# by256/icsg3d

Hardware: AMD Instinct MI355X
Metric: voxel-grids/s (fwd+bwd) for 32^3 U-Net+VAE at batch 32: value = U-Net train step (BASELINE configs[1]); DFC-VAE step (configs[2]) in secondary; both per batch in unet_plus_vae (higher is better)
Workload: dtype f32

## Files before the change

icsg3d_amd/csrc/common.h:

```cpp
#pragma once
#include <hip/hip_runtime.h>
#include <hip/hip_ext.h>
#include <atomic>
#include <cstdint>
#include <cstdio>
#include <string>
#include <vector>

#include "up8.h"
#include "up125.h"

namespace ics {

extern std::atomic<long long> g_kernel_launches;
struct LaunchTimer {
  virtual void next(hipEvent_t* start, hipEvent_t* stop) = 0;
  virtual ~LaunchTimer() = default;
};
extern thread_local LaunchTimer* tl_launch_timer;
template <typename... P, typename... A>
inline void ics_launch(void (*kernel)(P...), dim3 grid, dim3 block, size_t shmem, hipStream_t st, A&&... args) {
  static_assert(sizeof...(P) == sizeof...(A), "kernel argument count");
  if (tl_launch_timer != nullptr) {
    hipEvent_t e0 = nullptr, e1 = nullptr;
    tl_launch_timer->next(&e0, &e1);
    hipExtLaunchKernelGGL(kernel, grid, block, (std::uint32_t)shmem, st, e0, e1, 0u, static_cast<P>(args)...);
  } else {
    hipLaunchKernelGGL(kernel, grid, block, shmem, st, static_cast<P>(args)...);
  }
}
#define ICS_LAUNCH(...)                                      \
  do {                                                       \
    ::ics::g_kernel_launches.fetch_add(1, std::memory_order_relaxed); \
    ::ics::ics_launch(__VA_ARGS__);                          \
  } while (0)

void set_error(const std::string& msg);
#define ICS_HIP(expr)                                                                     \
  do {                                                                                    \
    hipError_t _e = (expr);                                                               \
    if (_e != hipSuccess) {                                                               \
      ::ics::set_error(std::string(#expr) + " -> " + hipGetErrorString(_e) + " @" +       \
                       __FILE__ + ":" + std::to_string(__LINE__));                        \
      return -1;                                                                          \
    }                                                                                     \
  } while (0)
#define ICS_CHECK(cond, msg)                                                              \
  do {                                                                                    \
    if (!(cond)) {                                                                        \
      ::ics::set_error(std::string(msg) + " (" #cond ") @" + __FILE__ + ":" +             \
                       std::to_string(__LINE__));                                         \
      return -1;                                                                          \
    }                                                                                     \
  } while (0)
#define ICS_TRY(expr)                                                                     \
  do {                                                                                    \
    if ((expr) != 0) return -1;                                                           \
  } while (0)

enum Act : int { ACT_NONE = 0, ACT_RELU = 1, ACT_LRELU = 2 };
constexpr float kLeaky = 0.3f;
constexpr float kBnEps = 1e-3f;
constexpr float kKEps = 1e-7f;
constexpr float kPoolTieTol = 1e-5f;

__device__ __forceinline__ float act_fwd(float v, int act) {
  if (act == ACT_RELU) return fmaxf(v, 0.f);
  if (act == ACT_LRELU) return v > 0.f ? v : kLeaky * v;
  return v;
}
__device__ __forceinline__ float act_grad(float v, int act) {
  if (act == ACT_RELU) return v > 0.f ? 1.f : 0.f;
  if (act == ACT_LRELU) return v > 0.f ? 1.f : kLeaky;
  return 1.f;
}

struct ConvSrc {
  const float* p;
  const float* scale;
  const float* shift;
  int C;
  int up;
  int act;
  int bcast;
};

enum ConvFlags : int {
  CF_NO_REUSE = 1,
  CF_NO_WGRAD3 = 2,
  CF_NO_WGRAD3S = 4,
  CF_NO_FWD_SPLITK = 8,
  CF_NO_THIN_N = 16,
  CF_NO_UPSPLIT = 32,
  CF_NO_THIN_C = 64,
  CF_NO_COND_FOLD = 128,
  CF_NO_WINO = 256,
  CF_NO_WINO_WGRAD = 512,
  CF_NO_WINO64 = 1024,
  CF_NO_UP3 = 2048,
  CF_NO_THIN1_2STAGE = 4096,
  CF_NO_FAST_BNBWD = 8192,
  CF_NO_FUSED_HEAD = 16384,
  CF_NO_BWD_FOLD = 32768,
  CF_UP3_BIG_ALWAYS = 65536,
  CF_NO_WINOG = 262144,
  CF_NO_HEAD_BNFUSE = 524288,
  CF_NO_UP3N = 1 << 21,
  CF_NO_DGRAD_BNFUSE = 1 << 22,
  CF_NO_POOL_PRESUM = 1 << 23,
  CF_NO_HEAD_LABELS = 1 << 24,
  CF_NO_UP8 = 1 << 25,
  CF_UP8 = 1 << 26,
  CF_NO_UP125 = 1 << 27,
  CF_FORCE_UP125 = 1 << 28,
  CF_POOL125_V1 = 1 << 29,
  CF_ZBATCH = 1 << 20,
};
int conv_flags_from_env();

struct ConvGeom {
  int B, S, lgS;
  int Cin, Cout;
  int taps;
  int Kpad, Npad;
  int flags = 0;
};

struct BwdStat {
  const float* s = nullptr;
  const float* mean = nullptr;
  const float* rstd = nullptr;
  const float* scale = nullptr;
  const float* shift = nullptr;
  float* partial = nullptr;
  int post_act = ACT_NONE;
  int ld = 0;
  const float* abc = nullptr;
  float* db_partial = nullptr;
  const float* pool_d = nullptr;
  int pool_ld = 0;
  const unsigned char* pool_mask = nullptr;
};

int launch_conv_fwd(hipStream_t st, const ConvGeom& g, const ConvSrc* src, int nsrc,
                    const float* wpacked, const float* bias, float* out, int ldo, int pre_act,
                    float* stat_partial, int* stat_rows_per_block, int accumulate = 0,
                    float* splitk_ws = nullptr, size_t splitk_ws_floats = 0, const BwdStat* bwd = nullptr,
                    int* bwd_blocks = nullptr);
size_t conv_fwd_workspace_floats(const ConvGeom& g, const ConvSrc* src, int nsrc);
bool conv_fwd_up8_tile_ok(const ConvGeom& g);
bool conv_thin_c_ok(const ConvGeom& g, const ConvSrc& s0, int nsrc, int cin_log);
size_t conv_thin_c_wgrad_workspace_floats(const ConvGeom& g);
int launch_conv_wgrad_thin_c(hipStream_t st, const ConvGeom& g, const ConvSrc& s0, const float* dy, int ldy, float* dw,
                             int ldw, int row_pitch, float* ws, size_t ws_floats, int phase);
int launch_conv_fwd_thin_c(hipStream_t st, const ConvGeom& g, const ConvSrc& s0, int cin_log, int wstride,
                           const float* wp, const float* bias, float* out, int ldo, int pre_act, float* stat_partial,
                           int* rows_per_block, const float* pos_bias = nullptr);
int launch_conv_fwd_par(hipStream_t st, const ConvGeom& g_lowres, const ConvSrc& src, const float* wpar, float* out,
                        int ldo, const float* bias = nullptr, int pre_act = ACT_NONE, float* stat_partial = nullptr,
                        int* stat_blocks = nullptr);
int launch_pack_par(hipStream_t st, const float* w, int Cin_total, int Cout, int c_off, int Cu, float* dst, int Kpad,
                    int Npad);
int launch_pack_fwd_sub(hipStream_t st, const float* w, int taps, int Cin_total, int Cout, int c_off, int Csub,
                        float* dst, int Kpad, int Npad);
int launch_conv_wgrad(hipStream_t st, const ConvGeom& g, const ConvSrc* src, int nsrc,
                      const float* dy, int ldy, float* dw, int ldw, float* workspace,
                      size_t workspace_floats, int sub_rows = 0, int row_pitch = 0, int row_off = 0,
                      int phase = 0);
const char* conv_last_kernel_id();
void conv_set_last_kernel_id(const char* id);
int launch_pack_sub(hipStream_t st, const float* w, int taps, int Cin_total, int Cout, int c_off, int Csub,
                    int flip, float* dst, int Kpad, int Npad);
size_t conv_wgrad_workspace_floats(const ConvGeom& g, const ConvSrc* src, int nsrc);
int conv_fwd_rows_per_block(const ConvGeom& g);
int launch_conv_wgrad_ablate(hipStream_t st, const ConvGeom& g, const ConvSrc* src, const float* dy, int ldy,
                             float* workspace, int ablate);
int launch_conv_fwd_ablate(hipStream_t st, const ConvGeom& g, const ConvSrc* src, int nsrc, const float* wp,
                           float* out, int ldo, int ablate);
int launch_pack_fwd(hipStream_t st, const float* w, int K, int N, float* dst, int Kpad, int Npad,
                    int k_off, int n_off, int zero_first, int cin_log = 0, int cin_phys = 0);
void* pack_table_record_begin();
int pack_table_record_end(void* handle, std::vector<unsigned char>* bytes, int* njobs, unsigned* nblocks);
int launch_pack_table(hipStream_t st, const void* d_jobs, int njobs, unsigned nblocks);
int launch_materialize_input(hipStream_t st, const ConvSrc* src, int nsrc, int Cin, int CinG, int B, int S,
                             float* out);
int launch_pack_bwd(hipStream_t st, const float* w, int taps, int Cin, int Cout, float* dst,
                    int Kpad, int Npad, int cout_total, int co_off, int zero_first);

bool conv_wino_ok(const ConvGeom& g, const ConvSrc* src, int nsrc);
size_t conv_wino_weight_floats(int Cin, int Cout);
int launch_conv_fwd_wino(hipStream_t st, const ConvGeom& g, const ConvSrc& s0, const float* wt, const float* bias,
                         float* out, int ldo, int pre_act, float* stat_partial, int* rows_per_block, int accumulate,
                         int layout, const BwdStat* bwd = nullptr, int* bwd_blocks = nullptr);
int launch_pack_wino(hipStream_t st, const float* w, int Cin_total, int Cout, int c_off, int Csub, int bwd, float* dst,
                     int layout = 0);
int conv_wino_layout(const ConvGeom& g);
bool conv_wino64_ok(const ConvGeom& g, const ConvSrc* src, int nsrc);
int launch_conv_fwd_wino64(hipStream_t st, const ConvGeom& g, const ConvSrc& s0, const float* wt, const float* bias,
                           float* out, int ldo, int pre_act, float* stat_partial, int* rows_per_block, int accumulate,
                           const BwdStat* bwd = nullptr, int* bwd_blocks = nullptr);
bool conv_wino_wgrad_ok(const ConvGeom& g, const ConvSrc* src, int nsrc);
size_t conv_wino_wgrad_workspace_floats(const ConvGeom& g);
int launch_conv_wgrad_wino(hipStream_t st, const ConvGeom& g, const ConvSrc& s0, const float* dy, int ldy, float* dw,
                           int ldw, float* ws, size_t ws_floats, int sub_rows, int row_pitch, int row_off, int phase);
bool conv_up3_ok(const ConvGeom& g, const ConvSrc& s0);
size_t conv_up3_weight_floats(int Cu, int Cout);
int launch_pack_up3(hipStream_t st, const float* w, int Cin_total, int Cout, int c_off, int Cu, float* dst);
int launch_conv_fwd_up3(hipStream_t st, const ConvGeom& g, const ConvSrc& s0, const float* wt, const float* bias,
                        float* out, int ldo, int pre_act, float* stat_partial, int* stat_blocks, int accumulate);
bool conv_winog_ok(const ConvGeom& g, const ConvSrc* src, int nsrc);
bool conv_winog_wgrad_ok(const ConvGeom& g, const ConvSrc* src, int nsrc);
size_t conv_winog_weight_floats(int Cin, int Cout);
void conv_winog_scratch_floats(const ConvGeom& g, size_t* v, size_t* m, size_t* z);
int launch_conv_fwd_winog(hipStream_t st, const ConvGeom& g, const ConvSrc& s0, const float* wg, const float* bias, float* out,
                          int ldo, int pre_act, float* stat_partial, int* rows_per_block, float* v_scratch, float* m_scratch,
                          float* vt_keep);
int launch_conv_wgrad_winog(hipStream_t st, const ConvGeom& g, const float* vt, const float* dy, int ldy, float* dw, int ldw,
                            int row_pitch, int row_off, float* z_scratch, float* m_scratch);
int launch_gemm_zbatch(hipStream_t st, int nz, int M, int K, int N, const float* A, const float* Wp, float* out, int flags);
int wgrad_zbatch_splits(int nz, int M, int K, int N);
int launch_wgrad_zbatch(hipStream_t st, int nz, int M, int K, int N, const float* x, const float* dy, float* ws, int ksplit);
int launch_pack_up125(hipStream_t st, const float* w, int Cin_total, int N, int c_off, int Cu, float* dst);
int launch_pack_up125_pieces(hipStream_t st, const float* w, int Cin_total, int N, int c_off, int Cu, float* dst);
bool conv_up3n_ok(const ConvGeom& g, const ConvSrc& s0);
size_t conv_up3n_weight_floats(int Cu, int Cout);
int launch_pack_up3n(hipStream_t st, const float* w, int Cin_total, int Cout, int c_off, int Cu, float* dst);
int launch_conv_fwd_up3n(hipStream_t st, const ConvGeom& g, const ConvSrc& s0, const float* wt, const float* bias, float* out,
                         int ldo, int pre_act, float* stat_partial, int* stat_blocks);
int launch_wgrad_reduce_splits(hipStream_t st, const float* ws, int nsplit, size_t n_elems, int N, float* dw, int ldw,
                               int sub_rows, int row_pitch, int row_off);

}
```

icsg3d_amd/csrc/conv_igemm.hip:

```cpp
#include "common.h"

#ifndef ICS_GEMM_DEEP_FWD_MIN
#define ICS_GEMM_DEEP_FWD_MIN 1
#endif
#ifndef ICS_GEMM_DEEP_MIN
#define ICS_GEMM_DEEP_MIN 3
#endif
#ifndef ICS_GEMM_DEEP
#define ICS_GEMM_DEEP 1
#endif

#include <algorithm>
#include <type_traits>
#include <cstdlib>
#include <cstring>
#include <vector>

namespace ics {

typedef float f32x16 __attribute__((ext_vector_type(16)));
typedef float v4f __attribute__((ext_vector_type(4)));

#ifndef ICS_KLDA
#define ICS_KLDA 36
#endif
constexpr int kLDA = ICS_KLDA;

__device__ __forceinline__ int xcd_swizzle(int bid, int nblk) {
  const int xcd = bid & 7, q = nblk >> 3, r = nblk & 7;
  return (xcd < r ? xcd * (q + 1) : r * (q + 1) + (xcd - r) * q) + (bid >> 3);
}

static thread_local const char* g_last_kernel_id = "";
const char* conv_last_kernel_id() { return g_last_kernel_id; }
void conv_set_last_kernel_id(const char* id) { g_last_kernel_id = id; }
static const char* tf(bool b) { return b ? "true" : "false"; }

int conv_flags_from_env() {
  int f = 0;
  if (getenv("ICSG3D_NO_REUSE")) f |= CF_NO_REUSE;
  if (getenv("ICSG3D_NO_WGRAD3")) f |= CF_NO_WGRAD3;
  if (getenv("ICSG3D_NO_WGRAD3S")) f |= CF_NO_WGRAD3S;
  if (getenv("ICSG3D_NO_FWD_SPLITK")) f |= CF_NO_FWD_SPLITK;
  if (getenv("ICSG3D_NO_THIN_N")) f |= CF_NO_THIN_N;
  if (getenv("ICSG3D_NO_UPSPLIT")) f |= CF_NO_UPSPLIT;
  if (getenv("ICSG3D_NO_THIN_C")) f |= CF_NO_THIN_C;
  if (getenv("ICSG3D_NO_COND_FOLD")) f |= CF_NO_COND_FOLD;
  if (getenv("ICSG3D_NO_WINO")) f |= CF_NO_WINO;
  if (getenv("ICSG3D_NO_WINO_WGRAD")) f |= CF_NO_WINO_WGRAD;
  if (getenv("ICSG3D_NO_WINO64")) f |= CF_NO_WINO64;
  if (getenv("ICSG3D_NO_UP3")) f |= CF_NO_UP3;
  if (getenv("ICSG3D_NO_THIN1_2STAGE")) f |= CF_NO_THIN1_2STAGE;
  if (getenv("ICSG3D_NO_FAST_BNBWD")) f |= CF_NO_FAST_BNBWD;
  if (getenv("ICSG3D_NO_FUSED_HEAD")) f |= CF_NO_FUSED_HEAD;
  if (getenv("ICSG3D_NO_BWD_FOLD")) f |= CF_NO_BWD_FOLD;
  if (getenv("ICSG3D_NO_WINOG")) f |= CF_NO_WINOG;
  if (getenv("ICSG3D_NO_HEAD_BNFUSE")) f |= CF_NO_HEAD_BNFUSE;
  if (getenv("ICSG3D_NO_UP3N")) f |= CF_NO_UP3N;
  if (getenv("ICSG3D_NO_DGRAD_BNFUSE")) f |= CF_NO_DGRAD_BNFUSE;
  if (getenv("ICSG3D_NO_POOL_PRESUM")) f |= CF_NO_POOL_PRESUM;
  if (getenv("ICSG3D_NO_HEAD_LABELS")) f |= CF_NO_HEAD_LABELS;
  if (getenv("ICSG3D_NO_UP8")) f |= CF_NO_UP8;
  if (getenv("ICSG3D_NO_UP125")) f |= CF_NO_UP125;
  if (getenv("ICSG3D_FORCE_UP125")) f |= CF_FORCE_UP125;
  if (getenv("ICSG3D_POOL125_V1")) f |= CF_POOL125_V1;
  { const char* e = getenv("ICSG3D_UP3_BIG_MIN_WG"); if (e && *e && strtoul(e, nullptr, 10) <= 1) f |= CF_UP3_BIG_ALWAYS; }
  return f;
}
struct DevOnce {
  bool done[64] = {false};
  bool need(int* dev) {
    int d = 0;
    if (hipGetDevice(&d) != hipSuccess || d < 0 || d >= 64) { *dev = -1; return true; }
    *dev = d;
    return !done[d];
  }
  void mark(int dev) { if (dev >= 0) done[dev] = true; }
};

static int identity_affine(const float** ones, const float** zeros) {
  constexpr int kN = 16384;
  static float* buf[64] = {nullptr};
  int dev = 0;
  ICS_HIP(hipGetDevice(&dev));
  ICS_CHECK(dev >= 0 && dev < 64, "device index out of range");
  if (!buf[dev]) {
    float* p = nullptr;
    ICS_HIP(hipMalloc(&p, 2 * kN * sizeof(float)));
    std::vector<float> h(2 * kN, 0.f);
    for (int i = 0; i < kN; ++i) h[i] = 1.f;
    ICS_HIP(hipMemcpy(p, h.data(), 2 * kN * sizeof(float), hipMemcpyHostToDevice));
    buf[dev] = p;
  }
  *ones = buf[dev];
  *zeros = buf[dev] + kN;
  return 0;
}
static int fix_src(ConvSrc& s) {
  if (s.scale == nullptr) {
    ICS_CHECK(s.C <= 16384, "source wider than the identity-affine buffer");
    ICS_TRY(identity_affine(&s.scale, &s.shift));
    s.act = ACT_NONE;
  }
  return 0;
}

struct RowPos {
  int b, z, y, x;
};
__device__ __forceinline__ RowPos decode_row(int m, int S, int lg) {
  RowPos r;
  r.x = m & (S - 1);
  r.y = (m >> lg) & (S - 1);
  r.z = (m >> (2 * lg)) & (S - 1);
  r.b = m >> (3 * lg);
  return r;
}

__device__ __forceinline__ size_t src_voxel(const ConvSrc& s, int b, int z, int y, int x, int S) {
  if (s.up) {
    const int Sh = S >> 1;
    return ((((size_t)b * Sh + (z >> 1)) * Sh + (y >> 1)) * Sh + (x >> 1)) * (size_t)s.C;
  }
  return ((((size_t)b * S + z) * S + y) * S + x) * (size_t)s.C;
}

__host__ __device__ __forceinline__ float act_slope_of(int act) {
  return act == ACT_RELU ? 0.f : (act == ACT_LRELU ? kLeaky : 1.f);
}
__device__ __forceinline__ float act_apply(float v, float slope) {
  return fmaxf(v, v * slope);
}
template <bool NOACT>
__device__ __forceinline__ v4f affine_only_or_act4(v4f v, v4f sc, v4f sh, float slope);
__device__ __forceinline__ v4f affine_act4(v4f v, v4f sc, v4f sh, float slope) {
  v4f r;
  r.x = act_apply(fmaf(v.x, sc.x, sh.x), slope); r.y = act_apply(fmaf(v.y, sc.y, sh.y), slope);
  r.z = act_apply(fmaf(v.z, sc.z, sh.z), slope); r.w = act_apply(fmaf(v.w, sc.w, sh.w), slope);
  return r;
}
template <bool NOACT>
__device__ __forceinline__ v4f affine_only_or_act4(v4f v, v4f sc, v4f sh, float slope) {
  if (!NOACT) return affine_act4(v, sc, sh, slope);
  v4f r;
  r.x = fmaf(v.x, sc.x, sh.x); r.y = fmaf(v.y, sc.y, sh.y); r.z = fmaf(v.z, sc.z, sh.z); r.w = fmaf(v.w, sc.w, sh.w);
  return r;
}
__device__ __forceinline__ unsigned voxel_off(int b, int z, int y, int x, int S, int u, int C) {
  const int Ss = S >> u;
  return ((((unsigned)b * Ss + (z >> u)) * Ss + (y >> u)) * Ss + (x >> u)) * (unsigned)C;
}
__device__ __forceinline__ int clampi(int v, int hi) { return min(max(v, 0), hi); }

__device__ __forceinline__ ConvSrc pick_src(const ConvSrc& s0, const ConvSrc& s1, bool first) {
  ConvSrc s;
  s.p = first ? s0.p : s1.p;
  s.scale = first ? s0.scale : s1.scale;
  s.shift = first ? s0.shift : s1.shift;
  s.C = first ? s0.C : s1.C;
  s.up = first ? s0.up : s1.up;
  s.act = first ? s0.act : s1.act;
  s.bcast = first ? s0.bcast : s1.bcast;
  return s;
}

__device__ __forceinline__ float gather_scalar(const ConvSrc& s0, const ConvSrc& s1, int ci, int b,
                                               int z, int y, int x, int S) {
  const bool first = ci < s0.C;
  const ConvSrc s = pick_src(s0, s1, first);
  const int cl = first ? ci : ci - s0.C;
  float v;
  if (s.bcast > 0) {
    v = s.p[(size_t)b * s.bcast + (cl % s.bcast)];
  } else {
    v = s.p[src_voxel(s, b, z, y, x, S) + cl];
  }
  if (s.scale) v = act_fwd(fmaf(v, s.scale[cl], s.shift[cl]), s.act);
  return v;
}

template <int WM, int WN, int TM, int TN, bool VEC, int ABL = 0, bool AFF = true, bool UP = true, bool THIN = false,
          bool REUSE = false, bool PAR = false, bool NOACT = false, bool FOLD = false, bool UP8 = false>
__global__ __launch_bounds__(256, FOLD ? 2 : ((REUSE && PAR) ? 3 : 1)) void conv_fwd_kernel(ConvGeom g, ConvSrc s0, ConvSrc s1,
                                                        const float* __restrict__ wp,
                                                        const float* __restrict__ bias,
                                                        float* __restrict__ out, int ldo, int pre_act,
                                                        float* __restrict__ stat_partial, int gridM,
                                                        int gridN, int accumulate, BwdStat bs, Up8Geom u8) {
  constexpr int BM = WM * TM * 32, BN = WN * TN * 32;
  constexpr int B_FLOATS = 32 * BN;
  constexpr int RA = BM / 32;
  constexpr int RS = BM / 8;
  constexpr int NB = BN / 32;
  extern __shared__ __attribute__((aligned(16))) float smem[];
  const int A_FLOATS = (REUSE ? BM + (BM >> g.lgS) + 1 : BM) * kLDA;
  float* As = smem;
  constexpr int NABUF = 1;
  float* Bs = smem + NABUF * A_FLOATS;

  const int t = threadIdx.x, lane = t & 63, wave = t >> 6;
  const int wm = wave / WN, wn = wave % WN;
  const int li = lane & 31, lh = lane >> 5;
  const int sw = xcd_swizzle(blockIdx.x, gridM * gridN);
  const int mb = sw / gridN, nb = sw % gridN;
  const int S = g.S, lg = g.lgS;
  const int M = g.B << (3 * lg);
  const int n0 = nb * BN;
  const int nchunks = g.Kpad >> 5;
  const int cpt = (VEC && !THIN) ? (g.Cin >> 5) : 1;
  const int cls = PAR ? (int)blockIdx.y : 0;
  const int pz = cls >> 2, py = (cls >> 1) & 1, px = cls & 1;
  if (PAR) wp += (size_t)cls * g.Kpad * g.Npad;
  const bool zbatch = (g.flags & CF_ZBATCH) != 0;
  if (zbatch) {
    s0.p += (size_t)blockIdx.z * (size_t)M * (size_t)s0.C;
    wp += (size_t)blockIdx.z * (size_t)g.Kpad * (size_t)g.Npad;
    out += (size_t)blockIdx.z * (size_t)M * (size_t)ldo;
  }
  const int zsplit = zbatch ? 1 : (int)gridDim.z, zidx = zbatch ? 0 : (int)blockIdx.z;

  const int mrow_base = mb * BM + (VEC ? (t >> 3) : (t >> 5));
  const float slope0 = act_slope_of(s0.act), slope1 = act_slope_of(s1.act);
  const float pre_slope = act_slope_of(pre_act);

  unsigned rmask[RA];
  int rvh[RA];
  if (VEC) {
#pragma unroll
    for (int r = 0; r < RA; ++r) {
      const int m = mrow_base + 32 * r;
      const RowPos rp = decode_row(m, S, lg);
      unsigned mk = 0;
      if (m < M) {
        if (PAR) {
#pragma unroll
          for (int tp = 0; tp < 8; ++tp) {
            const int zz = rp.z + (tp >> 2) + pz - 1, yy = rp.y + ((tp >> 1) & 1) + py - 1, xx = rp.x + (tp & 1) + px - 1;
            const bool ok = (unsigned)zz < (unsigned)S && (unsigned)yy < (unsigned)S && (unsigned)xx < (unsigned)S;
            mk |= (ok ? 1u : 0u) << tp;
          }
#pragma unroll
          for (int gz = 0; gz < 4; ++gz) {
            const int zz = rp.z + (gz >> 1) + pz - 1, yy = rp.y + (gz & 1) + py - 1;
            mk |= (((unsigned)zz < (unsigned)S && (unsigned)yy < (unsigned)S) ? 1u : 0u) << (8 + gz);
          }
        } else if (g.taps == 27) {
          const unsigned zm = (rp.z > 0 ? 1u : 0u) | 2u | (rp.z < S - 1 ? 4u : 0u);
          const unsigned ym = (rp.y > 0 ? 1u : 0u) | 2u | (rp.y < S - 1 ? 4u : 0u);
          const unsigned xm = (rp.x > 0 ? 1u : 0u) | 2u | (rp.x < S - 1 ? 4u : 0u);
#pragma unroll
          for (int tp = 0; tp < 27; ++tp)
            mk |= (((zm >> (tp / 9)) & (ym >> ((tp / 3) % 3)) & (xm >> (tp % 3))) & 1u) << tp;
        } else {
          mk = 1u;
        }
      }
      mk |= ((unsigned)(rp.z & 1) << 29) | ((unsigned)(rp.y & 1) << 28) | ((unsigned)(rp.x & 1) << 27);
      rmask[r] = mk;
      const int Sh = S >> 1;
      rvh[r] = ((rp.b * Sh + (rp.z >> 1)) * Sh + (rp.y >> 1)) * Sh + (rp.x >> 1);
    }
  }

  v4f ra4[RA];
  float ras[RS];
  v4f rb[NB];

  unsigned bofs[NB];
#pragma unroll
  for (int r = 0; r < NB; ++r) {
    const int idx = t + 256 * r;
    bofs[r] = (unsigned)((idx / BN) * g.Npad + n0 + idx % BN) * 16u;
  }
  auto load_b = [&](int krow4) {
    const char* wrow = reinterpret_cast<const char*>(wp) + (size_t)krow4 * (size_t)g.Npad * 16;
#pragma unroll
    for (int r = 0; r < NB; ++r) rb[r] = *reinterpret_cast<const v4f*>(wrow + bofs[r]);
  };
  auto store_b = [&](int buf) {
    float* Bw = Bs + buf * B_FLOATS;
#pragma unroll
    for (int r = 0; r < NB; ++r) *reinterpret_cast<v4f*>(Bw + (t + 256 * r) * 4) = rb[r];
  };
  unsigned rowB0[RA], rowB1[RA];
  if (VEC) {
#pragma unroll
    for (int r = 0; r < RA; ++r) {
      rowB0[r] = (unsigned)(mrow_base + 32 * r) * (unsigned)s0.C * 4u;
      rowB1[r] = (unsigned)(mrow_base + 32 * r) * (unsigned)s1.C * 4u;
    }
  }
  auto load_a_group = [&](int gzy, int cc) {
    const int ci0 = cc << 5;
    const int dz = PAR ? (gzy >> 1) + pz - 1 : gzy / 3 - 1, dy = PAR ? (gzy & 1) + py - 1 : gzy % 3 - 1;
    const bool first = ci0 < s0.C;
    const char* sp = reinterpret_cast<const char*>(first ? s0.p : s1.p);
    const float* sscale = first ? s0.scale : s1.scale;
    const float* sshift = first ? s0.shift : s1.shift;
    const int sC = first ? s0.C : s1.C, su = first ? s0.up : s1.up;
    const float slope = first ? slope0 : slope1;
    const int cl = (first ? ci0 : ci0 - s0.C) + (t & 7) * 4;
    const v4f sc = *reinterpret_cast<const v4f*>(sscale + cl);
    const v4f sh = *reinterpret_cast<const v4f*>(sshift + cl);
    const int sdelta = (dz * S + dy) * S;
    const unsigned goffb = (unsigned)(sdelta * sC + cl) * 4u;
    const int Sh = S >> 1;
#pragma unroll
    for (int r = 0; r < RA; ++r) {
      const unsigned mk = rmask[r];
      const bool inb = (mk >> (PAR ? 8 + gzy : gzy * 3 + 1)) & 1u;
      unsigned offb = (first ? rowB0[r] : rowB1[r]) + goffb;
      if (UP) {
        const int ez = (dz + (int)((mk >> 29) & 1u)) >> 1;
        const int ey = (dy + (int)((mk >> 28) & 1u)) >> 1;
        const unsigned up_b = ((unsigned)(rvh[r] + (ez * Sh + ey) * Sh) * (unsigned)sC + (unsigned)cl) * 4u;
        offb = su ? up_b : offb;
      }
      offb = inb ? offb : (unsigned)cl * 4u;
      v4f v = *reinterpret_cast<const v4f*>(sp + offb);
      if (AFF) v = affine_only_or_act4<NOACT>(v, sc, sh, slope);
      ra4[r] = inb ? v : v4f{0.f, 0.f, 0.f, 0.f};
    }
  };
  auto store_a_group = [&](int buf) {
    float* A = As + buf * A_FLOATS;
#pragma unroll
    for (int r = 0; r < RA; ++r) {
      const int row = (t >> 3) + 32 * r;
      *reinterpret_cast<v4f*>(A + (row + (row >> lg) + 1) * kLDA + (t & 7) * 4) = ra4[r];
    }
  };

  auto load_chunk = [&](int c) {
    load_b(c * 8);
    if (VEC) {
      int tap, ci0;
      bool kvalid = true;
      if (THIN) {
        const int kq = (c << 5) + (t & 7) * 4;
        const int lgC = 31 - __clz(g.Cin);
        tap = kq >> lgC; ci0 = kq & (g.Cin - 1);
        kvalid = tap < g.taps;
      } else {
        tap = c / cpt; ci0 = (c - tap * cpt) << 5;
      }
      const bool t27 = g.taps == 27;
      int dz = t27 ? tap / 9 - 1 : 0, dy = t27 ? (tap / 3) % 3 - 1 : 0, dx = t27 ? tap % 3 - 1 : 0;
      if (PAR) { dz = (tap >> 2) + pz - 1; dy = ((tap >> 1) & 1) + py - 1; dx = (tap & 1) + px - 1; }
      const bool first = THIN ? true : (ci0 < s0.C);
      const float* sp = first ? s0.p : s1.p;
      const float* sscale = first ? s0.scale : s1.scale;
      const float* sshift = first ? s0.shift : s1.shift;
      const int sC = first ? s0.C : s1.C, su = first ? s0.up : s1.up;
      const float slope = first ? slope0 : slope1;
      const int cl = THIN ? ci0 : (first ? ci0 : ci0 - s0.C) + (t & 7) * 4;
      const v4f sc = *reinterpret_cast<const v4f*>(sscale + cl);
      const v4f sh = *reinterpret_cast<const v4f*>(sshift + cl);
      const int sdelta = (dz * S + dy) * S + dx;
      const int Sh = S >> 1;
#pragma unroll
      for (int r = 0; r < RA; ++r) {
        const unsigned mk = rmask[r];
        const bool inb = kvalid && ((mk >> (tap & 31)) & 1u);
        int idx = mrow_base + 32 * r + sdelta;
        if (UP) {
          const int ez = (dz + (int)((mk >> 29) & 1u)) >> 1;
          const int ey = (dy + (int)((mk >> 28) & 1u)) >> 1;
          const int ex = (dx + (int)((mk >> 27) & 1u)) >> 1;
          const int idx_up = rvh[r] + (ez * Sh + ey) * Sh + ex;
          idx = su ? idx_up : idx;
// ... 304 lines not shown
      __syncthreads();
    }
  } else {
    for (int c = 0; c + 1 < nchunks; ++c) {
      if (ABL == 1) compute(c & 1);
      else compute_regs_only();
      __syncthreads();
    }
  }
  compute((ce - 1) & 1);
  __syncthreads();
  }
  }
  if (zsplit > 1) out += (size_t)zidx * (size_t)M * ldo;

  const int mrow0 = mb * BM + wm * TM * 32 + 4 * lh;
  if (FOLD) {
    float* red1 = smem;
    float* red2 = smem + WM * BN;
#pragma unroll
    for (int j = 0; j < TN; ++j) {
      const int n = n0 + wn * TN * 32 + j * 32 + li;
      const bool nvalid = n < g.Cout;
      const int nc = nvalid ? n : 0;
      const float b_mu = bs.mean[nc], b_rs = bs.rstd[nc];
      const float b_sc = bs.post_act != ACT_NONE ? bs.scale[nc] : 1.f;
      const float b_sh = bs.post_act != ACT_NONE ? bs.shift[nc] : 0.f;
      float a1 = 0.f, a2 = 0.f;
      const char* sbase = reinterpret_cast<const char*>(bs.s);
      char* obase = reinterpret_cast<char*>(out);
      const unsigned s_ldb = (unsigned)bs.ld * 4u, o_ldb = (unsigned)ldo * 4u, colb = (unsigned)nc * 4u;
#pragma unroll
      for (int i = 0; i < TM; ++i) {
        float sv[16];
#pragma unroll
        for (int r = 0; r < 16; ++r) {
          const unsigned m = (unsigned)(mrow0 + i * 32 + (r & 3) + 8 * (r >> 2));
          sv[r] = *reinterpret_cast<const float*>(sbase + min(m, (unsigned)(M - 1)) * s_ldb + colb);
        }
#pragma unroll
        for (int r = 0; r < 16; ++r) {
          const unsigned m = (unsigned)(mrow0 + i * 32 + (r & 3) + 8 * (r >> 2));
          const bool ok = m < (unsigned)M && nvalid;
          const float v = acc[i][j][r];
          const float d = ok ? v * act_grad(fmaf(sv[r], b_sc, b_sh), bs.post_act) : 0.f;
          a1 += d;
          a2 = fmaf(d, (sv[r] - b_mu) * b_rs, a2);
          if (ok) *reinterpret_cast<float*>(obase + m * o_ldb + colb) = v;
        }
        asm volatile("" ::: "memory");
      }
      a1 += __shfl_xor(a1, 32);
      a2 += __shfl_xor(a2, 32);
      if (lh == 0) {
        red1[wm * BN + wn * TN * 32 + j * 32 + li] = a1;
        red2[wm * BN + wn * TN * 32 + j * 32 + li] = a2;
      }
    }
    __syncthreads();
    if (t < BN) {
      float a1 = 0.f, a2 = 0.f;
#pragma unroll
      for (int w = 0; w < WM; ++w) { a1 += red1[w * BN + t]; a2 += red2[w * BN + t]; }
      float* sp = bs.partial + (size_t)(n0 + t) * gridM + mb;
      sp[0] = a1;
      sp[(size_t)g.Npad * gridM] = a2;
    }
    return;
  }
  float colsum[TN];
#pragma unroll
  for (int j = 0; j < TN; ++j) {
    const int n = n0 + wn * TN * 32 + j * 32 + li;
    const bool nvalid = n < g.Cout;
    const float bv = (bias != nullptr && nvalid) ? bias[n] : 0.f;
    float cs = 0.f;
#pragma unroll
    for (int i = 0; i < TM; ++i)
#pragma unroll
      for (int r = 0; r < 16; ++r) {
        const int m = mrow0 + i * 32 + (r & 3) + 8 * (r >> 2);
        const bool ok = m < M;
        size_t mo = m;
        if (PAR) {
          const RowPos rp = decode_row(m, S, lg);
          mo = ((((size_t)rp.b * (2 * S) + 2 * rp.z + pz) * (2 * S) + 2 * rp.y + py) * (2 * S)) + 2 * rp.x + px;
        }
        float a = acc[i][j][r] + bv;
        if (PAR && accumulate && ok && nvalid) a += out[mo * ldo + n];
        float v = act_apply(a, pre_slope);
        if (!ok) v = 0.f;
        acc[i][j][r] = v;
        cs += v;
        if (ok && nvalid) out[mo * ldo + n] = v;
      }
    colsum[j] = cs;
  }
  if (stat_partial == nullptr) return;

  float* red = smem;
  float* bmean = smem + WM * BN;
  const int nvalid_rows = min(BM, M - mb * BM);
#pragma unroll
  for (int j = 0; j < TN; ++j) {
    float cs = colsum[j];
    cs += __shfl_xor(cs, 32);
    if (lh == 0) red[wm * BN + wn * TN * 32 + j * 32 + li] = cs;
  }
  __syncthreads();
  if (t < BN) {
    float s = 0.f;
#pragma unroll
    for (int w = 0; w < WM; ++w) s += red[w * BN + t];
    bmean[t] = s / (float)nvalid_rows;
  }
  __syncthreads();
#pragma unroll
  for (int j = 0; j < TN; ++j) {
    const float mu = bmean[wn * TN * 32 + j * 32 + li];
    float q = 0.f;
#pragma unroll
    for (int i = 0; i < TM; ++i)
#pragma unroll
      for (int r = 0; r < 16; ++r) {
        const int m = mrow0 + i * 32 + (r & 3) + 8 * (r >> 2);
        const float d = acc[i][j][r] - mu;
        q += (m < M) ? d * d : 0.f;
      }
    q += __shfl_xor(q, 32);
    colsum[j] = q;
  }
  __syncthreads();
#pragma unroll
  for (int j = 0; j < TN; ++j)
    if (lh == 0) red[wm * BN + wn * TN * 32 + j * 32 + li] = colsum[j];
  __syncthreads();
  if (t < BN) {
    float q = 0.f;
#pragma unroll
    for (int w = 0; w < WM; ++w) q += red[w * BN + t];
    const size_t nstat = (size_t)(PAR ? 8 : 1) * gridM;
    float* sp = stat_partial + (size_t)(n0 + t) * nstat + (size_t)(cls * gridM + mb);
    sp[0] = (float)nvalid_rows;
    sp[(size_t)g.Npad * nstat] = bmean[t];
    sp[(size_t)2 * g.Npad * nstat] = q;
  }
}

template <int WM, int WN, int TM, int TN, bool VEC, int ABL = 0, bool AFF = true, bool UP = true, bool THIN = false,
          bool REUSE = false, bool PAR = false, bool NOACT = false, bool FOLD = false, bool UP8 = false>
static int launch_fwd_cfg(hipStream_t st, const ConvGeom& g, const ConvSrc& s0, const ConvSrc& s1,
                          const float* wp, const float* bias, float* out, int ldo, int pre_act,
                          float* stat_partial, int* rows_per_block, int accumulate = 0, int ksplit = 1,
                          const BwdStat* bwd = nullptr) {
  constexpr int BM = WM * TM * 32, BN = WN * TN * 32;
  const int M = g.B << (3 * g.lgS);
  const int gridM = (M + BM - 1) / BM, gridN = g.Npad / BN;
  const int arows = REUSE ? BM + (BM >> g.lgS) + 1 : BM;
  const size_t lds = (size_t)(arows * kLDA + 2 * 32 * BN) * sizeof(float);
  auto kern = conv_fwd_kernel<WM, WN, TM, TN, VEC, ABL, AFF, UP, THIN, REUSE, PAR, NOACT, FOLD, UP8>;
  static DevOnce attr;
  int dev;
  if (attr.need(&dev)) {
    const size_t lds_max = (size_t)((REUSE ? BM + BM / 4 + 1 : BM) * kLDA + 2 * 32 * BN) * sizeof(float);
    ICS_HIP(hipFuncSetAttribute(reinterpret_cast<const void*>(kern),
                                hipFuncAttributeMaxDynamicSharedMemorySize, (int)lds_max));
    attr.mark(dev);
  }
  if (rows_per_block) *rows_per_block = BM;
  static const std::string id = std::string("conv_fwd_kernel<") + std::to_string(WM) + ", " + std::to_string(WN) + ", " +
                                std::to_string(TM) + ", " + std::to_string(TN) + ", " + tf(VEC) + ", " +
                                std::to_string(ABL) + ", " + tf(AFF) + ", " + tf(UP) + ", " + tf(THIN) + ", " +
                                tf(REUSE) + ", " + tf(PAR) + ", " + tf(NOACT) + ", " + tf(FOLD) + (UP8 ? ", UP8>" : ">");
  g_last_kernel_id = id.c_str();
  BwdStat bs_arg;
  if (FOLD) bs_arg = *bwd;
  Up8Geom u8;
  if (UP8) u8 = up8_geom(g.B, g.S, g.lgS, g.Cin / 27);
  ICS_LAUNCH(kern, dim3(gridM * gridN, PAR ? 8 : 1, ksplit), dim3(256), lds, st, g, s0, s1, wp, bias, out, ldo,
                     pre_act, stat_partial, gridM, gridN, accumulate, bs_arg, u8);
  ICS_HIP(hipGetLastError());
  return 0;
}

static void pick_fwd_tile(const ConvGeom& g, int* bm, int* bn) {
  const int M = g.B << (3 * g.lgS);
  int BN = (g.Npad % 128 == 0) ? 128 : (g.Npad % 96 == 0) ? 96 : (g.Npad % 64 == 0) ? 64 : 32;
  int BM = 128;
  if (g.Npad % 64 == 0 && (long)((M + 127) / 128) * (g.Npad / BN) < 384) {
    BM = 64;
    BN = 64;
  }
  *bm = BM;
  *bn = BN;
}

static bool up8_tile(int bm, int bn) { return bm == 64 || bn == 128 || bn == 64; }
bool conv_fwd_up8_tile_ok(const ConvGeom& g) {
  int bm, bn;
  pick_fwd_tile(g, &bm, &bn);
  return up8_tile(bm, bn);
}

static bool fwd_is_vec(const ConvGeom& g, const ConvSrc& s0, const ConvSrc& s1) {
  return (g.Cin % 32 == 0) && (s0.C % 32 == 0) && s0.bcast == 0 && s1.bcast == 0;
}
static bool conv_is_thin(const ConvGeom& g, const ConvSrc& s0, int nsrc) {
  return nsrc == 1 && s0.bcast == 0 && s0.C == g.Cin && (g.Cin == 4 || g.Cin == 8 || g.Cin == 16);
}


int launch_gemm_zbatch(hipStream_t st, int nz, int M, int K, int N, const float* A, const float* Wp, float* out, int flags) {
  ICS_CHECK(nz >= 1 && nz <= 65535 && M >= 1 && K % 32 == 0 && N % 64 == 0, "z-batched GEMM: K % 32, N % 64 required");
  ICS_CHECK((size_t)M * (size_t)std::max(K, N) < ((size_t)1 << 30), "z-batched GEMM: matrix too large for 32-bit offsets");
  const ConvGeom g{M, 1, 0, K, N, 1, K, N, flags | CF_ZBATCH};
  const ConvSrc s0{A, nullptr, nullptr, K, 0, ACT_NONE, 0}, s1{};
#ifndef ICS_ZB_BIG
#define ICS_ZB_BIG 1
#endif
  if (ICS_ZB_BIG && M % 128 == 0 && N % 128 == 0 && (long)(M / 128) * (N / 128) * nz >= 512)
    return launch_fwd_cfg<2, 2, 2, 2, true, 0, false, false, false, false, false, true, false>(
        st, g, s0, s1, Wp, nullptr, out, N, ACT_NONE, nullptr, nullptr, 0, nz);
  return launch_fwd_cfg<2, 2, 1, 1, true, 0, false, false, false, false, false, true, false>(
      st, g, s0, s1, Wp, nullptr, out, N, ACT_NONE, nullptr, nullptr, 0, nz);
}

int conv_fwd_rows_per_block(const ConvGeom& g) {
  int bm, bn;
  pick_fwd_tile(g, &bm, &bn);
  if (g.taps == 27 && g.Cout <= 4 && g.Cin % 4 == 0 && g.Cin >= 4 && g.Cin <= 64) {
    bm = std::min(bm, g.Cin <= 16 ? 256 : 64);
  }
  return bm;
}

#ifndef ICS_THINC_UNROLL
#define ICS_THINC_UNROLL 3
#endif
template <int CIN, int COUT>
__global__ __launch_bounds__(256) void conv_thin_c_fwd_kernel(ConvGeom g, const float* __restrict__ x, int wstride,
                                                               const float* __restrict__ wp,
                                                               const float* __restrict__ bias,
                                                               float* __restrict__ out, int ldo, int pre_act,
                                                               float* __restrict__ stat_partial,
                                                               const float* __restrict__ pos_bias) {
  constexpr int LPV = COUT / 4;
  constexpr int GPB = 256 / LPV;
  constexpr int VPB = 4 * GPB;
  constexpr int C4 = CIN >= 4 ? CIN / 4 : 1;
  extern __shared__ __attribute__((aligned(16))) float smem[];
  float* w = smem;
  const int t = threadIdx.x;
  const int S = g.S, lg = g.lgS;
  const int M = g.B << (3 * lg);
  constexpr bool WCH = CIN < 4;
  const int wrow = WCH ? 1 : wstride;
  const int K = 27 * wrow;
  for (int i = t; i < K * COUT; i += 256) {
    const int kk = i / COUT, n = i - kk * COUT;
    const int k = WCH ? kk * wstride : kk;
    w[i] = wp[((size_t)(k >> 2) * g.Npad + n) * 4 + (k & 3)];
  }
  __syncthreads();
  const int q = t % LPV, grp = t / LPV;
  const int m0 = ((int)blockIdx.x * GPB + grp) * 4;
  const bool gvalid = m0 < M;
  const int x0 = m0 & (S - 1), y = (m0 >> lg) & (S - 1), z = (m0 >> (2 * lg)) & (S - 1);
  float acc[4][4];
#pragma unroll
  for (int v = 0; v < 4; ++v)
#pragma unroll
    for (int j = 0; j < 4; ++j) acc[v][j] = 0.f;
  const float* wq = w + 4 * q;
#pragma unroll ICS_THINC_UNROLL
  for (int gzy = 0; gzy < 9; ++gzy) {
    const int dz = gzy / 3 - 1, dy = gzy % 3 - 1;
    const bool rowok = gvalid && (unsigned)(z + dz) < (unsigned)S && (unsigned)(y + dy) < (unsigned)S;
    const long rowbase = (long)(m0 + (dz * S + dy) * S - 1) * CIN;
#pragma unroll
    for (int c4 = 0; c4 < C4; ++c4) {
      float xv[6][4];
#pragma unroll
      for (int p = 0; p < 6; ++p) {
        const bool ok = rowok && (unsigned)(x0 + p - 1) < (unsigned)S;
        if (CIN >= 4) {
          v4f tv = v4f{0.f, 0.f, 0.f, 0.f};
          if (ok) tv = *reinterpret_cast<const v4f*>(x + rowbase + (long)p * CIN + c4 * 4);
          xv[p][0] = tv.x; xv[p][1] = tv.y; xv[p][2] = tv.z; xv[p][3] = tv.w;
        } else {
          xv[p][0] = ok ? x[rowbase + p] : 0.f;
          xv[p][1] = xv[p][2] = xv[p][3] = 0.f;
        }
      }
#pragma unroll
      for (int dx = 0; dx < 3; ++dx) {
        const float* wk = wq + (size_t)((gzy * 3 + dx) * wrow + c4 * 4) * COUT;
#pragma unroll
        for (int j = 0; j < (CIN >= 4 ? 4 : 1); ++j) {
          const v4f wv = *reinterpret_cast<const v4f*>(wk + j * COUT);
#pragma unroll
          for (int v = 0; v < 4; ++v) {
            const float xs = xv[v + dx][j];
            acc[v][0] = fmaf(xs, wv.x, acc[v][0]); acc[v][1] = fmaf(xs, wv.y, acc[v][1]);
            acc[v][2] = fmaf(xs, wv.z, acc[v][2]); acc[v][3] = fmaf(xs, wv.w, acc[v][3]);
          }
        }
      }
    }
  }
  const float pre_slope = act_slope_of(pre_act);
  v4f bv = v4f{0.f, 0.f, 0.f, 0.f};
  if (bias != nullptr) { bv.x = bias[4 * q]; bv.y = bias[4 * q + 1]; bv.z = bias[4 * q + 2]; bv.w = bias[4 * q + 3]; }
  float csum[4] = {0.f, 0.f, 0.f, 0.f};
  const int bsmp = m0 >> (3 * lg);
  const int czy = ((z == 0 ? 0 : (z == S - 1 ? 2 : 1)) * 3 + (y == 0 ? 0 : (y == S - 1 ? 2 : 1))) * 3;
#pragma unroll
  for (int v = 0; v < 4; ++v) {
    if (pos_bias != nullptr && gvalid) {
      const int xx = x0 + v;
      const int cls = czy + (xx == 0 ? 0 : (xx == S - 1 ? 2 : 1));
      const float* pb = pos_bias + ((size_t)bsmp * 27 + cls) * COUT + 4 * q;
      bv.x = pb[0]; bv.y = pb[1]; bv.z = pb[2]; bv.w = pb[3];
    }
    acc[v][0] = act_apply(acc[v][0] + bv.x, pre_slope); acc[v][1] = act_apply(acc[v][1] + bv.y, pre_slope);
    acc[v][2] = act_apply(acc[v][2] + bv.z, pre_slope); acc[v][3] = act_apply(acc[v][3] + bv.w, pre_slope);
    if (gvalid) {
      *reinterpret_cast<v4f*>(out + (size_t)(m0 + v) * ldo + 4 * q) = v4f{acc[v][0], acc[v][1], acc[v][2], acc[v][3]};
#pragma unroll
      for (int j = 0; j < 4; ++j) csum[j] += acc[v][j];
    } else {
#pragma unroll
      for (int j = 0; j < 4; ++j) acc[v][j] = 0.f;
    }
  }
  if (stat_partial == nullptr) return;
  __syncthreads();
  float* red = smem;
  float* bmean = smem + 4 * COUT;
  const int lane = t & 63, wave = t >> 6;
  const int nvalid = min(VPB, M - (int)blockIdx.x * VPB);
#pragma unroll
  for (int j = 0; j < 4; ++j) {
    float a = csum[j];
    for (int o = LPV; o < 64; o <<= 1) a += __shfl_xor(a, o);
    if (lane < LPV) red[wave * COUT + 4 * lane + j] = a;
  }
  __syncthreads();
  if (t < COUT) bmean[t] = (red[t] + red[COUT + t] + red[2 * COUT + t] + red[3 * COUT + t]) / (float)nvalid;
  __syncthreads();
  float mu[4], qs[4] = {0.f, 0.f, 0.f, 0.f};
#pragma unroll
  for (int j = 0; j < 4; ++j) mu[j] = bmean[4 * q + j];
  if (gvalid) {
#pragma unroll
    for (int v = 0; v < 4; ++v)
#pragma unroll
      for (int j = 0; j < 4; ++j) { const float d = acc[v][j] - mu[j]; qs[j] = fmaf(d, d, qs[j]); }
  }
  __syncthreads();
#pragma unroll
  for (int j = 0; j < 4; ++j) {
    float a = qs[j];
    for (int o = LPV; o < 64; o <<= 1) a += __shfl_xor(a, o);
    if (lane < LPV) red[wave * COUT + 4 * lane + j] = a;
  }
  __syncthreads();
  if (t < COUT) {
    const size_t nstat = gridDim.x;
    float* sp = stat_partial + (size_t)t * nstat + blockIdx.x;
    sp[0] = (float)nvalid;
    sp[(size_t)g.Npad * nstat] = bmean[t];
    sp[(size_t)2 * g.Npad * nstat] = red[t] + red[COUT + t] + red[2 * COUT + t] + red[3 * COUT + t];
  }
}

static int launch_reduce_splits(hipStream_t st, const float* ws, int nsplit, size_t n_elems, int N, float* dw, int ldw,
                                int sub_rows, int row_pitch, int row_off);
// ... 696 lines not shown
    if (variant == 1) return launch_fwd_cfg<WM, WN, TM, TN, true, 0, true, false>(ICS_FWD_ARGS);  \
    return launch_fwd_cfg<WM, WN, TM, TN, true, 0, true, true>(ICS_FWD_ARGS);                   \
  } while (0)
  if (bm == 64) { ICS_FWD(2, 2, 1, 1); }
  if (bn == 128) { ICS_FWD(2, 2, 2, 2); }
  if (bn == 96) { ICS_FWD(4, 1, 1, 3); }
  if (bn == 64) { ICS_FWD(2, 2, 2, 1); }
  ICS_FWD(4, 1, 1, 1);
#undef ICS_FWD_ARGS
#undef ICS_FWD
}

static void pick_par_tile(const ConvGeom& g, int* bm, int* bn) {
  pick_fwd_tile(g, bm, bn);
  if (*bm == 64 && g.Npad % 128 == 0 && (long)(((g.B << (3 * g.lgS)) + 127) / 128) * (g.Npad / 128) * 8 >= 384) {
    *bm = 128; *bn = 128;
  }
}
int launch_conv_fwd_par(hipStream_t st, const ConvGeom& g, const ConvSrc& src, const float* wp, float* out,
                        int ldo, const float* bias, int pre_act, float* stat_partial, int* stat_blocks) {
  ConvSrc s0 = src, s1 = src;
  s1.C = 0;
  ICS_CHECK(g.taps == 8 && g.Cin % 32 == 0 && s0.C == g.Cin && !s0.up && !s0.bcast && g.Kpad == 8 * g.Cin,
            "parity-class conv needs a direct 32k-channel source");
  ICS_TRY(fix_src(s0));
  ICS_TRY(fix_src(s1));
  int bm, bn;
  pick_par_tile(g, &bm, &bn);
  int rpb = 0;
#define ICS_PAR_ARGS st, g, s0, s1, wp, bias, out, ldo, pre_act, stat_partial, &rpb
  int rc;
  const bool no_reuse = (g.flags & CF_NO_REUSE) != 0;
  const bool reuse = !no_reuse && g.S >= 4 && g.S <= bm;
  const bool noact = src.scale != nullptr && src.act == ACT_NONE;
#define ICS_PAR(WM, WN, TM, TN)                                                                              \
  (reuse ? (noact ? launch_fwd_cfg<WM, WN, TM, TN, true, 0, true, false, false, true, true, true>(ICS_PAR_ARGS) \
                  : launch_fwd_cfg<WM, WN, TM, TN, true, 0, true, false, false, true, true>(ICS_PAR_ARGS))   \
         : launch_fwd_cfg<WM, WN, TM, TN, true, 0, true, false, false, false, true>(ICS_PAR_ARGS))
  if (bm == 64) rc = ICS_PAR(2, 2, 1, 1);
  else if (bn == 128) rc = ICS_PAR(2, 2, 2, 2);
  else if (bn == 96) rc = ICS_PAR(4, 1, 1, 3);
  else if (bn == 64) rc = ICS_PAR(2, 2, 2, 1);
  else rc = ICS_PAR(4, 1, 1, 1);
#undef ICS_PAR
#undef ICS_PAR_ARGS
  if (stat_blocks) *stat_blocks = 8 * (((g.B << (3 * g.lgS)) + rpb - 1) / rpb);
  return rc;
}

struct PackJob {
  int kind;
  const float* w;
  float* dst;
  int a[9];
  unsigned long long total;
  unsigned blk0;
};
static thread_local std::vector<PackJob>* g_pack_rec = nullptr;

__device__ __forceinline__ float pack_par_value(size_t i, const float* __restrict__ w, int Cin_total, int Cout, int c_off,
                                                int Cu, int Kpad, int Npad) {
  const size_t per = (size_t)Kpad * Npad;
  const int cls = (int)(i / per);
  const size_t j = i - (size_t)cls * per;
  const int tq = j & 3;
  const size_t rest = j >> 2;
  const int n = rest % Npad;
  const int k = (int)(rest / Npad) * 4 + tq;
  const int e = k / Cu, c = k - e * Cu;
  float v = 0.f;
  if (e < 8 && n < Cout) {
    const int p3[3] = {cls >> 2, (cls >> 1) & 1, cls & 1};
    const int e3[3] = {e >> 2, (e >> 1) & 1, e & 1};
    int lo[3], hi[3];
#pragma unroll
    for (int a = 0; a < 3; ++a) {
      if (p3[a] == 0) { lo[a] = e3[a] ? 1 : 0; hi[a] = e3[a] ? 2 : 0; }
      else { lo[a] = e3[a] ? 2 : 0; hi[a] = e3[a] ? 2 : 1; }
    }
    for (int dz = lo[0]; dz <= hi[0]; ++dz)
      for (int dy = lo[1]; dy <= hi[1]; ++dy)
        for (int dx = lo[2]; dx <= hi[2]; ++dx)
          v += w[((size_t)((dz * 3 + dy) * 3 + dx) * Cin_total + c_off + c) * Cout + n];
  }
  return v;
}
__global__ void pack_par_kernel(const float* __restrict__ w, int Cin_total, int Cout, int c_off, int Cu,
                                float* __restrict__ dst, int Kpad, int Npad) {
  const size_t i = (size_t)blockIdx.x * blockDim.x + threadIdx.x;
  if (i >= 8 * (size_t)Kpad * Npad) return;
  dst[i] = pack_par_value(i, w, Cin_total, Cout, c_off, Cu, Kpad, Npad);
}
int launch_pack_par(hipStream_t st, const float* w, int Cin_total, int Cout, int c_off, int Cu, float* dst,
                    int Kpad, int Npad) {
  if (g_pack_rec) { g_pack_rec->push_back(PackJob{4, w, dst, {Cin_total, Cout, c_off, Cu, Kpad, Npad, 0, 0, 0}, 8ull * Kpad * Npad, 0}); return 0; }
  const size_t total = (size_t)8 * Kpad * Npad;
  ICS_LAUNCH(pack_par_kernel, dim3((unsigned)((total + 255) / 256)), dim3(256), 0, st, w, Cin_total, Cout,
                     c_off, Cu, dst, Kpad, Npad);
  ICS_HIP(hipGetLastError());
  return 0;
}
__device__ __forceinline__ float pack_fwd_sub_value(size_t i, const float* __restrict__ w, int taps, int Cin_total,
                                                    int Cout, int c_off, int Csub, int Npad) {
  const int tq = i & 3;
  const size_t rest = i >> 2;
  const int n = rest % Npad;
  const int k = (int)(rest / Npad) * 4 + tq;
  const int tap = k / Csub, c = k - tap * Csub;
  return (tap < taps && n < Cout) ? w[((size_t)tap * Cin_total + c_off + c) * Cout + n] : 0.f;
}
__global__ void pack_fwd_sub_kernel(const float* __restrict__ w, int taps, int Cin_total, int Cout, int c_off,
                                    int Csub, float* __restrict__ dst, int Kpad, int Npad) {
  const size_t i = (size_t)blockIdx.x * blockDim.x + threadIdx.x;
  if (i >= (size_t)Kpad * Npad) return;
  dst[i] = pack_fwd_sub_value(i, w, taps, Cin_total, Cout, c_off, Csub, Npad);
}
int launch_pack_fwd_sub(hipStream_t st, const float* w, int taps, int Cin_total, int Cout, int c_off, int Csub,
                        float* dst, int Kpad, int Npad) {
  if (g_pack_rec) { g_pack_rec->push_back(PackJob{3, w, dst, {taps, Cin_total, Cout, c_off, Csub, Npad, 0, 0, 0}, (unsigned long long)Kpad * Npad, 0}); return 0; }
  const size_t total = (size_t)Kpad * Npad;
  ICS_LAUNCH(pack_fwd_sub_kernel, dim3((unsigned)((total + 255) / 256)), dim3(256), 0, st, w, taps,
                     Cin_total, Cout, c_off, Csub, dst, Kpad, Npad);
  ICS_HIP(hipGetLastError());
  return 0;
}

int launch_conv_fwd_ablate(hipStream_t st, const ConvGeom& g, const ConvSrc* src, int nsrc, const float* wp,
                           float* out, int ldo, int ablate) {
  ConvSrc s0 = src[0], s1 = src[nsrc > 1 ? 1 : 0];
  if (nsrc == 1) s1.C = 0;
  ICS_TRY(fix_src(s0));
  ICS_TRY(fix_src(s1));
  ICS_CHECK(fwd_is_vec(g, s0, s1) && g.Npad % 128 == 0, "ablation bench needs the vector 128x128 configuration");
#define ICS_ABL_ARGS st, g, s0, s1, wp, nullptr, out, ldo, 0, nullptr, nullptr
  if (ablate == 1) return launch_fwd_cfg<2, 2, 2, 2, true, 1, true, false>(ICS_ABL_ARGS);
  if (ablate == 2) return launch_fwd_cfg<2, 2, 2, 2, true, 2, true, false>(ICS_ABL_ARGS);
  if (ablate == 3) return launch_fwd_cfg<2, 2, 2, 2, true, 3, true, false>(ICS_ABL_ARGS);
  if (ablate == 4) return launch_fwd_cfg<2, 2, 2, 2, true, 4, true, false>(ICS_ABL_ARGS);
  if (ablate == 8) return launch_fwd_cfg<2, 2, 2, 2, true, 8, false, false>(ICS_ABL_ARGS);
  if (ablate == 9) return launch_fwd_cfg<2, 2, 2, 2, true, 9, false, false>(ICS_ABL_ARGS);
  if (ablate == 5) return launch_fwd_cfg<2, 2, 2, 2, true, 0, true, false>(ICS_ABL_ARGS);
  if (ablate == 6) return launch_fwd_cfg<2, 2, 2, 2, true, 0, true, true>(ICS_ABL_ARGS);
  return launch_fwd_cfg<2, 2, 2, 2, true, 0, false, false>(ICS_ABL_ARGS);
#undef ICS_ABL_ARGS
}


template <int WM, int WN, int TM, int TN, bool VEC, bool DYVEC, bool AFF = true, bool UP = true, bool THIN = false,
          int ABL = 0, bool UP8 = false, bool ZB = false>
__global__ __launch_bounds__(256) void conv_wgrad_kernel(ConvGeom g, ConvSrc s0, ConvSrc s1,
                                                          const float* __restrict__ dy, int ldy,
                                                          int n_load,
                                                          float* __restrict__ ws, int ktiles,
                                                          int ntiles, int rows_per_split, Up8Geom u8) {
  constexpr int KT = WM * TM * 32, NT = WN * TN * 32;
  constexpr int A_FLOATS = 32 * KT, D_FLOATS = 32 * NT;
  constexpr int AF4 = KT / 4, ATOT = 32 * AF4, APASS = ATOT / 256;
  constexpr int DF4 = NT / 4, DTOT = 32 * DF4, DPASS = DTOT / 256;
  static_assert(ATOT % 256 == 0 && DTOT % 256 == 0, "tile loads must divide evenly over 256 threads");
  extern __shared__ __attribute__((aligned(16))) float smem[];
  float* As = smem;
  float* Ds = smem + 2 * A_FLOATS;

  const int t = threadIdx.x, lane = t & 63, wave = t >> 6;
  const int wm = wave / WN, wn = wave % WN;
  const int li = lane & 31, lh = lane >> 5;
  const int S = g.S, lg = g.lgS;
  const int M = g.B << (3 * lg);
  const int K = g.taps * g.Cin;
  if (ZB) {
    s0.p += (size_t)blockIdx.y * (size_t)M * (size_t)s0.C;
    dy += (size_t)blockIdx.y * (size_t)M * (size_t)ldy;
    ws += (size_t)blockIdx.y * (size_t)(gridDim.x / (unsigned)(ktiles * ntiles)) * (size_t)K * (size_t)g.Cout;
  }

  int bid = blockIdx.x;
  const int nt_i = bid % ntiles; bid /= ntiles;
  const int kt_i = bid % ktiles; bid /= ktiles;
  const int split = bid;
  const int n0 = nt_i * NT;
  const int m_begin = split * rows_per_split;
  const int m_end = min(M, m_begin + rows_per_split);
  const int nchunks = (m_end - m_begin + 31) >> 5;

  const int k0 = kt_i * KT;
  int tdz = 0, tdy = 0, tdx = 0, sdelta = 0, xbad = -1, ybad = -1, zbad = -1;
  bool kvalid = false;
  const float* sp = s0.p;
  int sC = s0.C, su = 0, cl0 = 0;
  float slope = 1.f;
  v4f sc = v4f{1.f, 1.f, 1.f, 1.f}, sh = v4f{0.f, 0.f, 0.f, 0.f};
  if (VEC) {
    const int kf = k0 + (t % AF4) * 4;
    const int tap = kf / g.Cin, ci = kf - tap * g.Cin;
    kvalid = kf < K;
    if (g.taps == 27 && kvalid) { tdz = tap / 9 - 1; tdy = (tap / 3) % 3 - 1; tdx = tap % 3 - 1; }
    sdelta = (tdz * S + tdy) * S + tdx;
    xbad = tdx < 0 ? 0 : (tdx > 0 ? S - 1 : -1);
    ybad = tdy < 0 ? 0 : (tdy > 0 ? S - 1 : -1);
    zbad = tdz < 0 ? 0 : (tdz > 0 ? S - 1 : -1);
    const bool first = ci < s0.C;
    const ConvSrc sv = pick_src(s0, s1, first);
    sp = sv.p; sC = sv.C; su = sv.up;
    cl0 = kvalid ? (first ? ci : ci - s0.C) : 0;
    slope = act_slope_of(sv.act);
    if (AFF) {
      sc = *reinterpret_cast<const v4f*>(sv.scale + cl0);
      sh = *reinterpret_cast<const v4f*>(sv.shift + cl0);
    }
  }
  int s_tap = 0, s_ci = 0; bool s_kvalid = false; int sdz = 0, sdy = 0, sdx = 0;
  if (!VEC) {
    const int kf = k0 + (t & 31);
    s_tap = kf / g.Cin; s_ci = kf - s_tap * g.Cin; s_kvalid = kf < K;
    if (g.taps == 27) { sdz = s_tap / 9 - 1; sdy = (s_tap / 3) % 3 - 1; sdx = s_tap % 3 - 1; }
  }

  v4f ra[VEC ? APASS : 1];
  float ras[4];
  v4f rd[DPASS];

  auto load_chunk = [&](int c) {
    const int mbase = m_begin + (c << 5);
    if (VEC) {
      const int Sh = S >> 1;
#pragma unroll
      for (int p = 0; p < APASS; ++p) {
        const int m = mbase + (t + 256 * p) / AF4;
        const int x = m & (S - 1), y = (m >> lg) & (S - 1), z = (m >> (2 * lg)) & (S - 1);
        const bool inb = kvalid && m < m_end && x != xbad && y != ybad && z != zbad;
        int idx = m + sdelta;
        if (UP) {
          const int b = m >> (3 * lg);
          const int idx_up = ((b * Sh + ((z + tdz) >> 1)) * Sh + ((y + tdy) >> 1)) * Sh + ((x + tdx) >> 1);
          idx = su ? idx_up : idx;
        }
        const unsigned off = inb ? (unsigned)idx * (unsigned)sC + cl0 : (unsigned)cl0;
        v4f v = *reinterpret_cast<const v4f*>(sp + off);
        if (AFF) v = affine_act4(v, sc, sh, slope);
        ra[p] = inb ? v : v4f{0.f, 0.f, 0.f, 0.f};
      }
    } else {
#pragma unroll
      for (int p = 0; p < 4; ++p) {
        const int m = mbase + (t >> 5) + 8 * p;
        float v = 0.f;
        if (s_kvalid && m < m_end) {
          const RowPos r = decode_row(m, S, lg);
          const int zz = r.z + sdz, yy = r.y + sdy, xx = r.x + sdx;
          if ((unsigned)zz < (unsigned)S && (unsigned)yy < (unsigned)S && (unsigned)xx < (unsigned)S)
            v = gather_scalar(s0, s1, s_ci, r.b, zz, yy, xx, S);
        }
        ras[p] = v;
      }
    }
#pragma unroll
    for (int p = 0; p < DPASS; ++p) {
      const int idx = t + 256 * p;
      const int m = mbase + idx / DF4;
      const int n = n0 + (idx % DF4) * 4;
      const float* q = dy + (size_t)min(m, M - 1) * ldy;
      v4f v;
      if (DYVEC) {
        v = *reinterpret_cast<const v4f*>(q + min(n, n_load - 4));
        if (!(m < m_end && n < n_load)) v = v4f{0.f, 0.f, 0.f, 0.f};
      } else {
        v.x = q[min(n + 0, n_load - 1)]; v.y = q[min(n + 1, n_load - 1)];
        v.z = q[min(n + 2, n_load - 1)]; v.w = q[min(n + 3, n_load - 1)];
        const bool rowok = m < m_end;
        v.x = (rowok && n + 0 < n_load) ? v.x : 0.f; v.y = (rowok && n + 1 < n_load) ? v.y : 0.f;
        v.z = (rowok && n + 2 < n_load) ? v.z : 0.f; v.w = (rowok && n + 3 < n_load) ? v.w : 0.f;
      }
      rd[p] = v;
    }
  };
  const bool gemm = VEC && DYVEC && !UP && !THIN && ABL == 0 && g.taps == 1 && (M & 31) == 0 &&
                    (rows_per_split & 31) == 0 && (UP8 || n0 + NT <= n_load);
  const bool noact_g = slope == 1.f;
  unsigned aoffg[VEC ? APASS : 1], doffg[DPASS];
  if (VEC) {
#pragma unroll
    for (int p = 0; p < APASS; ++p) aoffg[p] = (unsigned)(((t + 256 * p) / AF4) * sC + cl0) * 4u;
  }
#pragma unroll
  for (int p = 0; p < DPASS; ++p) {
    const int idx = t + 256 * p;
    doffg[p] = UP8 ? (up8_prow((unsigned)(idx / DF4), u8.lgSh, u8.P) * (unsigned)u8.N +
                      up8_col_floats(min(n0 + (idx % DF4) * 4, n_load - 4), u8)) * 4u
                   : (unsigned)((idx / DF4) * ldy + n0 + (idx % DF4) * 4) * 4u;
  }
  auto load_chunk_gemm = [&](int c, auto noact_tag) {
    constexpr bool NA = decltype(noact_tag)::value;
    const int mbase = m_begin + (c << 5);
    const char* abase = reinterpret_cast<const char*>(sp) + (size_t)mbase * (size_t)sC * 4;
    const char* dbase = reinterpret_cast<const char*>(dy) +
                        (UP8 ? up8_chunk_base_floats((unsigned)mbase, u8) : (size_t)mbase * (size_t)ldy) * 4;
    if (VEC) {
#pragma unroll
      for (int p = 0; p < APASS; ++p) {
        v4f v = *reinterpret_cast<const v4f*>(abase + aoffg[p]);
        if (AFF) v = affine_only_or_act4<NA>(v, sc, sh, slope);
        ra[p] = v;
      }
    }
#pragma unroll
    for (int p = 0; p < DPASS; ++p) rd[p] = *reinterpret_cast<const v4f*>(dbase + doffg[p]);
  };
  auto store_chunk = [&](int buf) {
    float* A = As + buf * A_FLOATS;
    float* D = Ds + buf * D_FLOATS;
    if (VEC) {
#pragma unroll
      for (int p = 0; p < APASS; ++p) {
        const int idx = t + 256 * p;
        *reinterpret_cast<v4f*>(A + (idx / AF4) * KT + (idx % AF4) * 4) = ra[p];
      }
    } else {
#pragma unroll
      for (int p = 0; p < 4; ++p) A[((t >> 5) + 8 * p) * KT + (t & 31)] = ras[p];
    }
#pragma unroll
    for (int p = 0; p < DPASS; ++p) {
      const int idx = t + 256 * p;
      *reinterpret_cast<v4f*>(D + (idx / DF4) * NT + (idx % DF4) * 4) = rd[p];
    }
  };

  f32x16 acc[TM][TN];
#pragma unroll
// ... 463 lines not shown
  const int sC = first ? s0.C : s1.C;
  const float slope = act_slope_of(first ? s0.act : s1.act);
  const int ac4 = t & 15;
  const int cl = (first ? c0 : c0 - s0.C) + ac4 * 4;
  if (AFF && t < 32) {
    const float* src = (t < 16) ? (first ? s0.scale : s1.scale) : (first ? s0.shift : s1.shift);
    *reinterpret_cast<v4f*>(Aff + t * 4) = *reinterpret_cast<const v4f*>(src + (first ? c0 : c0 - s0.C) + (t & 15) * 4);
  }
  const unsigned aoff = (unsigned)((t >> 4) * sC + cl) * 4u;
  const unsigned hoff = (unsigned)cl * 4u;
  unsigned doff[4];
#pragma unroll
  for (int p = 0; p < 4; ++p) doff[p] = (unsigned)(((t >> 5) + 8 * p) * ldy + n0 + (t & 31) * 4) * 4u;
  const int hside = (t >> 4) & 1;

  v4f ra[2], rd[4], rah = v4f{0.f, 0.f, 0.f, 0.f};
  auto load_chunk = [&](int c) {
    const int mbase = m_begin + (c << 5);
    v4f sc = v4f{1.f, 1.f, 1.f, 1.f}, sh = v4f{0.f, 0.f, 0.f, 0.f};
    if (AFF) { sc = *reinterpret_cast<const v4f*>(Aff + ac4 * 4); sh = *reinterpret_cast<const v4f*>(Aff + 64 + ac4 * 4); }
#pragma unroll
    for (int p = 0; p < 2; ++p) {
      const int row0 = mbase + 16 * p;
      const int y = (row0 >> lg) & (S - 1), z = (row0 >> (2 * lg)) & (S - 1);
      const bool inb = (y != ybad) & (z != zbad);
      const float msk = inb ? 1.f : 0.f;
      const char* base = sp + (inb ? (long)(row0 + sdelta) * sC * 4 : 0L);
      v4f v = *reinterpret_cast<const v4f*>(base + aoff);
      if (AFF) v = affine_only_or_act4<NOACT>(v, sc, sh, slope);
      ra[p] = v4f{v.x * msk, v.y * msk, v.z * msk, v.w * msk};
    }
    if (halo) {
      const int x0 = mbase & (S - 1);
      const int y = (mbase >> lg) & (S - 1), z = (mbase >> (2 * lg)) & (S - 1);
      const bool lineok = (y != ybad) & (z != zbad);
      const bool inl = lineok & (x0 != 0), inr = lineok & (x0 == 0);
      const char* bl = sp + (inl ? (long)(mbase - 1 + sdelta) * sC * 4 : 0L);
      const char* br = sp + (inr ? (long)(mbase + 32 + sdelta) * sC * 4 : 0L);
      const float msk = (hside ? inr : inl) ? 1.f : 0.f;
      v4f v = *reinterpret_cast<const v4f*>((hside ? br : bl) + hoff);
      if (AFF) v = affine_only_or_act4<NOACT>(v, sc, sh, slope);
      rah = v4f{v.x * msk, v.y * msk, v.z * msk, v.w * msk};
    }
    const char* dbase = reinterpret_cast<const char*>(dy) + (size_t)mbase * (size_t)ldy * 4;
#pragma unroll
    for (int p = 0; p < 4; ++p) rd[p] = *reinterpret_cast<const v4f*>(dbase + doff[p]);
  };
  float* a_st[2];
#pragma unroll
  for (int p = 0; p < 2; ++p) {
    const int r = (t >> 4) + 16 * p;
    a_st[p] = As + (r + (halo ? 0 : (r >> lg)) + 1) * CK + ac4 * 4;
  }
  auto store_chunk = [&](int buf) {
#pragma unroll
    for (int p = 0; p < 2; ++p) *reinterpret_cast<v4f*>(a_st[p] + buf * A_FLOATS) = ra[p];
    if (halo && t < 32) *reinterpret_cast<v4f*>(As + buf * A_FLOATS + (hside ? 33 : 0) * CK + ac4 * 4) = rah;
    float* D = Ds + buf * D_FLOATS;
#pragma unroll
    for (int p = 0; p < 4; ++p) *reinterpret_cast<v4f*>(D + ((t >> 5) + 8 * p) * NT + (t & 31) * 4) = rd[p];
  };

  f32x16 acc[3][2];
#pragma unroll
  for (int i = 0; i < 3; ++i)
#pragma unroll
    for (int j = 0; j < 2; ++j)
#pragma unroll
      for (int r = 0; r < 16; ++r) acc[i][j][r] = 0.f;

  if (!halo) {
    for (int i = t; i < 2 * (lines + 1) * CK; i += 256) {
      const int b = i / ((lines + 1) * CK), rem = i - b * (lines + 1) * CK;
      As[b * A_FLOATS + (rem / CK) * (S + 1) * CK + rem % CK] = 0.f;
    }
  }
  __syncthreads();
  if (nchunks > 0) {
    load_chunk(0);
    store_chunk(0);
  }
  __syncthreads();
  auto compute = [&](int buf) {
    const float* A = As + buf * A_FLOATS + 2 * li + lh * CK;
    const float* D = Ds + buf * D_FLOATS + 32 * wave + li + lh * NT;
#pragma unroll
    for (int s = 0; s < 16; ++s) {
      constexpr int dummy = 0; (void)dummy;
      const int prow = 2 * s + (halo ? 0 : ((2 * s) >> lg)) + 1;
      const float b = D[(2 * s) * NT];
      float2 a[3];
#pragma unroll
      for (int dxi = 0; dxi < 3; ++dxi) a[dxi] = *reinterpret_cast<const float2*>(A + (prow + dxi - 1) * CK);
#pragma unroll
      for (int dxi = 0; dxi < 3; ++dxi) {
        acc[dxi][0] = __builtin_amdgcn_mfma_f32_32x32x2f32(a[dxi].x, b, acc[dxi][0], 0, 0, 0);
        acc[dxi][1] = __builtin_amdgcn_mfma_f32_32x32x2f32(a[dxi].y, b, acc[dxi][1], 0, 0, 0);
      }
    }
  };
  for (int c = 0; c + 1 < nchunks; ++c) {
    load_chunk(c + 1);
    compute(c & 1);
    store_chunk((c + 1) & 1);
    __syncthreads();
  }
  if (nchunks > 0) compute((nchunks - 1) & 1);

  float* wsp = ws + (size_t)split * K * g.Cout;
  const int n = n0 + 32 * wave + li;
#pragma unroll
  for (int dxi = 0; dxi < 3; ++dxi)
#pragma unroll
    for (int j = 0; j < 2; ++j)
#pragma unroll
      for (int r = 0; r < 16; ++r) {
        const int row = (r & 3) + 8 * (r >> 2) + 4 * lh;
        const int k = (gzy * 3 + dxi) * g.Cin + c0 + 2 * row + j;
        wsp[(size_t)k * g.Cout + n] = acc[dxi][j][r];
      }
}

static bool wgrad3_ok(const ConvGeom& g, const ConvSrc& s0, int nsrc, const ConvSrc& s1) {
  if ((g.flags & CF_NO_WGRAD3) || g.taps != 27 || g.S > 64 || g.S < 2 || g.Cin % 64 != 0 || g.Cout % 128 != 0) return false;
  if (s0.bcast || (nsrc > 1 && s1.bcast)) return false;
  if (nsrc > 1 && (s0.C % 64 != 0)) return false;
  return true;
}
struct Wgrad3Plan { int cgroups, ntiles, ksplit, rows_per_split; };
static Wgrad3Plan plan_wgrad3(const ConvGeom& g) {
  Wgrad3Plan p;
  const long M = (long)g.B << (3 * g.lgS);
  p.cgroups = g.Cin / 64;
  p.ntiles = g.Cout / 128;
  const int want = pick_ksplit(9L * p.cgroups * p.ntiles, M, g.lgS > 5 ? 512 : 768, 2);
  p.rows_per_split = (int)(((M + want - 1) / want + 31) / 32 * 32);
  p.ksplit = (int)((M + p.rows_per_split - 1) / p.rows_per_split);
  return p;
}


size_t conv_wgrad_workspace_floats(const ConvGeom& g, const ConvSrc* src, int nsrc) {
  if (thin_n_ok(g, src[0], nsrc)) return (size_t)thin_n_wgrad_splits(g) * g.taps * g.Cin * g.Cout;
  ConvSrc s0 = src[0], s1 = src[nsrc > 1 ? 1 : 0];
  WgradPlan p = plan_wgrad(g, s0, nsrc, s1);
  int ks = p.ksplit;
  if (wgrad3_ok(g, s0, nsrc, s1)) ks = std::max(ks, plan_wgrad3(g).ksplit);
  return (size_t)ks * g.taps * g.Cin * g.Cout;
}

template <int WM, int WN, int TM, int TN, bool VEC, bool DYVEC, bool AFF = true, bool UP = true, bool THIN = false,
          int ABL = 0, bool UP8 = false, bool ZB = false>
static int launch_wgrad_cfg(hipStream_t st, const ConvGeom& g, const ConvSrc& s0, const ConvSrc& s1,
                            const float* dy, int ldy, int n_load, float* ws, const WgradPlan& p, int nz = 1) {
  constexpr int KT = WM * TM * 32, NT = WN * TN * 32;
  const size_t lds = (size_t)2 * 32 * (KT + NT) * sizeof(float);
  auto kern = conv_wgrad_kernel<WM, WN, TM, TN, VEC, DYVEC, AFF, UP, THIN, ABL, UP8, ZB>;
  static DevOnce attr;
  int dev;
  if (attr.need(&dev)) {
    ICS_HIP(hipFuncSetAttribute(reinterpret_cast<const void*>(kern),
                                hipFuncAttributeMaxDynamicSharedMemorySize, (int)lds));
    attr.mark(dev);
  }
  static const std::string id = std::string("conv_wgrad_kernel<") + std::to_string(WM) + ", " + std::to_string(WN) +
                                ", " + std::to_string(TM) + ", " + std::to_string(TN) + ", " + tf(VEC) + ", " +
                                tf(DYVEC) + ", " + tf(AFF) + ", " + tf(UP) + ", " + tf(THIN) + ", " +
                                std::to_string(ABL) + (UP8 ? ", UP8>" : (ZB ? ", ZB>" : ">"));
  g_last_kernel_id = id.c_str();
  Up8Geom u8;
  if (UP8) u8 = up8_geom(g.B, g.S, g.lgS, g.Cout / 27);
  ICS_LAUNCH(kern, dim3(p.ktiles * p.ntiles * p.ksplit, ZB ? nz : 1), dim3(256), lds, st, g, s0, s1, dy,
                     ldy, n_load, ws, p.ktiles, p.ntiles, p.rows_per_split, u8);
  ICS_HIP(hipGetLastError());
  return 0;
}

int launch_conv_wgrad_ablate(hipStream_t st, const ConvGeom& g, const ConvSrc* src, const float* dy, int ldy,
                             float* workspace, int ablate) {
  ConvSrc s0 = src[0], s1 = src[0];
  s1.C = 0;
  ICS_TRY(fix_src(s0));
  ICS_TRY(fix_src(s1));
  WgradPlan p = plan_wgrad(g, s0, 1, s1);
  ICS_CHECK(p.vec && p.kt == 128 && p.nt == 128, "ablation bench needs the vector 128x128 configuration");
  if (ablate == 1) return launch_wgrad_cfg<2, 2, 2, 2, true, true, false, false, false, 1>(st, g, s0, s1, dy, ldy, g.Cout, workspace, p);
  return launch_wgrad_cfg<2, 2, 2, 2, true, true, false, false, false, 2>(st, g, s0, s1, dy, ldy, g.Cout, workspace, p);
}

int launch_conv_wgrad(hipStream_t st, const ConvGeom& g, const ConvSrc* src, int nsrc,
                      const float* dy, int ldy, float* dw, int ldw, float* workspace,
                      size_t workspace_floats, int sub_rows, int row_pitch, int row_off, int phase) {
  if (thin_n_ok(g, src[0], nsrc)) {
    const int ns = thin_n_wgrad_splits(g);
    const size_t n_el = (size_t)g.taps * g.Cin * g.Cout;
    ICS_CHECK((size_t)ns * n_el <= workspace_floats, "wgrad workspace too small");
    const int M = g.B << (3 * g.lgS);
    const int rows = (M + ns - 1) / ns;
    const int K = 27 * g.Cin;
    const bool aff = src[0].scale != nullptr;
    if (thin1_wgrad_ok(g, src[0])) {
      const int nb = thin1_wgrad_blocks(g);
      if (phase != 2) {
#define ICS_T1W(CKV)                                                                                                 \
  do {                                                                                                               \
    if (aff) ICS_LAUNCH((thin1_wgrad_kernel<CKV, true>), dim3(nb), dim3(256), 0, st, g, src[0], dy, ldy, workspace); \
    else ICS_LAUNCH((thin1_wgrad_kernel<CKV, false>), dim3(nb), dim3(256), 0, st, g, src[0], dy, ldy, workspace);    \
  } while (0)
        switch (g.Cin / 16) { case 1: ICS_T1W(1); break; case 2: ICS_T1W(2); break; case 3: ICS_T1W(3); break; default: ICS_T1W(4); break; }
#undef ICS_T1W
        ICS_HIP(hipGetLastError());
        g_last_kernel_id = "thin1_wgrad_kernel";
      }
      if (phase != 1) ICS_TRY(launch_reduce_splits(st, workspace, 4 * nb, n_el, g.Cout, dw, ldw, sub_rows, row_pitch, row_off));
      return 0;
    }
    if (phase != 2) {
#define ICS_TNW(NOUT, AFFV, KPT, NAME)                                                                         \
  do {                                                                                                         \
    g_last_kernel_id = NAME;                                                                                   \
    ICS_LAUNCH((conv_thin_n_wgrad_kernel<NOUT, AFFV, KPT>), dim3((M + rows - 1) / rows), dim3(256), 0,  \
                       st, g, src[0], dy, ldy, workspace, rows);                                               \
  } while (0)
#define ICS_TNW_K(NOUT, AFFV, TAG)                                                                  \
  do {                                                                                              \
    if (K <= 512) ICS_TNW(NOUT, AFFV, 2, "conv_thin_n_wgrad_kernel<" TAG ", 2>");                   \
    else if (K <= 1024) ICS_TNW(NOUT, AFFV, 4, "conv_thin_n_wgrad_kernel<" TAG ", 4>");             \
    else ICS_TNW(NOUT, AFFV, 7, "conv_thin_n_wgrad_kernel<" TAG ", 7>");                            \
  } while (0)
      if (g.Cout == 1) { if (aff) ICS_TNW_K(1, true, "1, true"); else ICS_TNW_K(1, false, "1, false"); }
      else { if (aff) ICS_TNW_K(4, true, "4, true"); else ICS_TNW_K(4, false, "4, false"); }
#undef ICS_TNW_K
#undef ICS_TNW
      ICS_HIP(hipGetLastError());
    }
    if (phase != 1)
      ICS_TRY(launch_reduce_splits(st, workspace, (M + rows - 1) / rows, n_el, g.Cout, dw, ldw, sub_rows, row_pitch,
                                   row_off));
    return 0;
  }
  ConvSrc s0 = src[0], s1 = src[nsrc > 1 ? 1 : 0];
  if (nsrc == 1) s1.C = 0;
  ICS_TRY(fix_src(s0));
  ICS_TRY(fix_src(s1));
  WgradPlan p = plan_wgrad(g, s0, nsrc, s1);
  const size_t n_elems = (size_t)g.taps * g.Cin * g.Cout;
  const int n_load4 = (g.Cout + 3) / 4 * 4;
  const bool dy_vec = (ldy % 4 == 0) && ((reinterpret_cast<uintptr_t>(dy) & 15) == 0) && (n_load4 <= ldy);
  const int n_load = dy_vec ? n_load4 : g.Cout;
  if (!dy_vec) {
    p.nt = (p.kt == 128) ? 32 : (p.kt == 64) ? 64 : 128;
    p.ntiles = (g.Npad + p.nt - 1) / p.nt;
  }
  const bool aff = src[0].scale != nullptr || (nsrc > 1 && src[1].scale != nullptr);
  const bool up = src[0].up || (nsrc > 1 && src[1].up);
  if (dy_vec && wgrad3_ok(g, s0, nsrc, s1)) {
    const Wgrad3Plan q = plan_wgrad3(g);
    ICS_CHECK((size_t)q.ksplit * n_elems <= workspace_floats, "wgrad workspace too small");
    const int arows = 32 + std::max(32 >> g.lgS, 1) + 1;
    const size_t lds = (size_t)(2 * (arows * 64 + 32 * 128) + 128) * sizeof(float);
    const dim3 grid(9 * q.cgroups * q.ntiles * q.ksplit);
    const int M3 = g.B << (3 * g.lgS);
    const bool fast = !up && g.lgS >= 4 && g.lgS <= 6 && M3 % 32 == 0 && n_load == g.Cout &&
                      !(g.flags & CF_NO_WGRAD3S);
    if (phase != 2 && fast) {
      const bool noact = aff && (src[0].scale == nullptr || src[0].act == ACT_NONE) &&
                         (nsrc < 2 || src[1].scale == nullptr || src[1].act == ACT_NONE);
      const int ar = 32 + (g.lgS == 6 ? 1 : (32 >> g.lgS)) + 1;
      const size_t lds3 = (size_t)(2 * (ar * 64 + 32 * 128) + 128) * sizeof(float);
#define ICS_W3S(AFFV, NOACTV, LGV)                                                                              \
  do {                                                                                                          \
    g_last_kernel_id = "conv_wgrad3s_kernel<" #AFFV ", " #NOACTV ", " #LGV ">";                                 \
    ICS_LAUNCH((conv_wgrad3s_kernel<AFFV, NOACTV, LGV>), grid, dim3(256), lds3, st, g, s0, s1, dy, ldy,  \
                       workspace, q.cgroups, q.ntiles, q.rows_per_split);                                       \
  } while (0)
#define ICS_W3S_L(AFFV, NOACTV)                                                       \
  do {                                                                                \
    if (g.lgS == 4) ICS_W3S(AFFV, NOACTV, 4);                                         \
    else if (g.lgS == 5) ICS_W3S(AFFV, NOACTV, 5);                                    \
    else ICS_W3S(AFFV, NOACTV, 6);                                                    \
  } while (0)
      if (!aff) ICS_W3S_L(false, false);
      else if (noact) ICS_W3S_L(true, true);
      else ICS_W3S_L(true, false);
#undef ICS_W3S_L
#undef ICS_W3S
      ICS_HIP(hipGetLastError());
    } else if (phase != 2) {
#define ICS_W3(AFFV, UPV, HALOV)                                                                                 \
  do {                                                                                                           \
    g_last_kernel_id = "conv_wgrad3_kernel<" #AFFV ", " #UPV ", " #HALOV ">";                                    \
    ICS_LAUNCH((conv_wgrad3_kernel<AFFV, UPV, HALOV>), grid, dim3(256), lds, st, g, s0, s1, dy, ldy,      \
                       n_load, workspace, q.cgroups, q.ntiles, q.rows_per_split);                                \
  } while (0)
      if (g.lgS > 5) {
        if (up) ICS_W3(true, true, true); else if (aff) ICS_W3(true, false, true); else ICS_W3(false, false, true);
      } else {
        if (up) ICS_W3(true, true, false); else if (aff) ICS_W3(true, false, false); else ICS_W3(false, false, false);
      }
#undef ICS_W3
      ICS_HIP(hipGetLastError());
    }
    if (phase != 1) {
      ICS_TRY(launch_reduce_splits(st, workspace, q.ksplit, n_elems, g.Cout, dw, ldw, sub_rows, row_pitch, row_off));
    }
    return 0;
  }
  ICS_CHECK((size_t)p.ksplit * n_elems <= workspace_floats, "wgrad workspace too small");
  if (phase != 2) {
#define ICS_WG_ARGS st, g, s0, s1, dy, ldy, n_load, workspace, p
#define ICS_WG(WM, WN, TM, TN, DV)                                                                 \
  do {                                                                                             \
    if (p.thin) ICS_TRY((launch_wgrad_cfg<WM, WN, TM, TN, true, DV, true, true, true>(ICS_WG_ARGS)));  \
    else if (!p.vec) ICS_TRY((launch_wgrad_cfg<WM, WN, TM, TN, false, DV, true, true>(ICS_WG_ARGS)));   \
    else if (up) ICS_TRY((launch_wgrad_cfg<WM, WN, TM, TN, true, DV, true, true>(ICS_WG_ARGS)));   \
    else if (aff) ICS_TRY((launch_wgrad_cfg<WM, WN, TM, TN, true, DV, true, false>(ICS_WG_ARGS))); \
    else ICS_TRY((launch_wgrad_cfg<WM, WN, TM, TN, true, DV, false, false>(ICS_WG_ARGS)));         \
  } while (0)
  if (g.flags & CF_UP8) {
    const int M8 = g.B << (3 * g.lgS);
    ICS_CHECK(dy_vec && p.vec && !p.thin && !up && g.taps == 1 && g.Cout % 27 == 0 && n_load == g.Cout && M8 % 32 == 0 &&
                  p.rows_per_split % 32 == 0 && up8_shape_ok(2 * g.S, g.Cout / 27, (size_t)M8, g.B),
              "up8 backward-weight: shape outside the 8-volume layout");
#define ICS_WG8(WM, WN, TM, TN)                                                                                  \
  do {                                                                                                           \
    if (aff) ICS_TRY((launch_wgrad_cfg<WM, WN, TM, TN, true, true, true, false, false, 0, true>(ICS_WG_ARGS)));  \
    else ICS_TRY((launch_wgrad_cfg<WM, WN, TM, TN, true, true, false, false, false, 0, true>(ICS_WG_ARGS)));     \
  } while (0)
    ICS_CHECK(p.nt == 128 && p.kt >= 64, "up8 backward-weight: no UP8 instantiation of this tile");
    if (p.kt == 128) ICS_WG8(2, 2, 2, 2);
    else ICS_WG8(2, 2, 1, 2);
#undef ICS_WG8
  } else if (!dy_vec) {
    if (p.kt == 128) ICS_WG(4, 1, 1, 1, false);
    else if (p.kt == 64) ICS_WG(2, 2, 1, 1, false);
    else ICS_WG(1, 4, 1, 1, false);
  } else if (p.kt == 128) {
    if (p.nt == 128) ICS_WG(2, 2, 2, 2, true);
    else if (p.nt == 96) ICS_WG(4, 1, 1, 3, true);
    else if (p.nt == 64) ICS_WG(4, 1, 1, 2, true);
    else ICS_WG(4, 1, 1, 1, true);
  } else if (p.kt == 64) {
    if (p.nt == 128) ICS_WG(2, 2, 1, 2, true);
    else ICS_WG(2, 2, 1, 1, true);
  } else {
    ICS_WG(1, 4, 1, 1, true);
  }
#undef ICS_WG_ARGS
#undef ICS_WG
  }
  if (phase != 1) {
    ICS_TRY(launch_reduce_splits(st, workspace, p.ksplit, n_elems, g.Cout, dw, ldw, sub_rows, row_pitch, row_off));
  }
  return 0;
}

int wgrad_zbatch_splits(int nz, int M, int K, int N) {
  const long base = (long)((K + 127) / 128) * ((N + 127) / 128) * nz;
  const long ks_max = std::max<long>(1, M / 256);
  return (int)std::max<long>(1, std::min<long>(std::min<long>(512 / base, ks_max), 512));
}
int launch_wgrad_zbatch(hipStream_t st, int nz, int M, int K, int N, const float* x, const float* dy, float* ws, int ksplit) {
  ICS_CHECK(nz >= 1 && nz <= 65535 && M >= 1 && K % 32 == 0 && N % 4 == 0 && ksplit >= 1, "z-batched wgrad: K % 32, N % 4 required");
  ICS_CHECK((size_t)M * (size_t)std::max(K, N) < ((size_t)1 << 30), "z-batched wgrad: matrix too large for 32-bit offsets");
  const ConvGeom g{M, 1, 0, K, N, 1, K, (N + 31) / 32 * 32, 0};
  const ConvSrc s0{x, nullptr, nullptr, K, 0, ACT_NONE, 0};
  ConvSrc s1 = s0;
  s1.C = 0;
  WgradPlan p;
  p.vec = true; p.thin = false;
  p.kt = 128; p.nt = 128;
  p.ktiles = (K + 127) / 128; p.ntiles = (N + 127) / 128;
  p.rows_per_split = ((M + ksplit - 1) / ksplit + 31) / 32 * 32;
  p.ksplit = (M + p.rows_per_split - 1) / p.rows_per_split;
  ICS_CHECK(p.ksplit <= ksplit, "z-batched wgrad: split plan");
  p.ksplit = ksplit;
  return launch_wgrad_cfg<2, 2, 2, 2, true, true, false, false, false, 0, false, true>(st, g, s0, s1, dy, N, N, ws, p, nz);
}

__device__ __forceinline__ bool pack_fwd_value(size_t i, const float* __restrict__ w, int K, int N, int Npad, int k_off,
                                               int n_off, int cin_log, int cin_phys, float* v) {
  const int tq = i & 3;
  const size_t rest = i >> 2;
  const int n = rest % Npad;
  const int k = (int)(rest / Npad) * 4 + tq;
  int ks = k - k_off;
  const int ns = n - n_off;
  bool ok = ks >= 0 && ks < K && ns >= 0 && ns < N;
  if (ok && cin_phys > 0) {
    const int tap = ks / cin_phys, ci = ks - tap * cin_phys;
    ok = ci < cin_log;
    ks = tap * cin_log + ci;
  }
  *v = ok ? w[(size_t)ks * N + ns] : 0.f;
  return ok;
}
__global__ void pack_fwd_kernel(const float* __restrict__ w, int K, int N, float* __restrict__ dst,
                                int Kpad, int Npad, int k_off, int n_off, int zero_first, int cin_log,
                                int cin_phys) {
  const size_t i = (size_t)blockIdx.x * blockDim.x + threadIdx.x;
  const size_t total = (size_t)Kpad * Npad;
  if (i >= total) return;
  float v;
  if (pack_fwd_value(i, w, K, N, Npad, k_off, n_off, cin_log, cin_phys, &v) || zero_first) dst[i] = v;
}

__global__ void materialize_input_kernel(ConvSrc s0, ConvSrc s1, int Cin, int CinG, int S, int lg, size_t total,
                                         float* __restrict__ out) {
  const size_t i = (size_t)blockIdx.x * blockDim.x + threadIdx.x;
  if (i >= total) return;
  const int c = (int)(i % CinG);
  const RowPos r = decode_row((int)(i / CinG), S, lg);
  out[i] = c < Cin ? gather_scalar(s0, s1, c, r.b, r.z, r.y, r.x, S) : 0.f;
}
int launch_materialize_input(hipStream_t st, const ConvSrc* src, int nsrc, int Cin, int CinG, int B, int S,
                             float* out) {
  ConvSrc s0 = src[0], s1 = src[nsrc > 1 ? 1 : 0];
  if (nsrc == 1) s1.C = 0;
  int lg = 0;
  while ((1 << lg) < S) ++lg;
  const size_t total = (size_t)B * S * S * S * CinG;
  ICS_LAUNCH(materialize_input_kernel, dim3((unsigned)((total + 255) / 256)), dim3(256), 0, st, s0, s1, Cin,
                     CinG, S, lg, total, out);
  ICS_HIP(hipGetLastError());
  return 0;
}

__device__ __forceinline__ bool pack_bwd_value(size_t i, const float* __restrict__ w, int taps, int Cin, int Cout,
                                               int Npad, int cout_total, int co_off, float* v) {
  const int tq = i & 3;
  const size_t rest = i >> 2;
  const int n = rest % Npad;
  const int k = (int)(rest / Npad) * 4 + tq;
  const int tp = k / cout_total, co = k - tp * cout_total - co_off;
  const bool ok = tp < taps && co >= 0 && co < Cout && n < Cin;
  *v = ok ? w[((size_t)(taps - 1 - tp) * Cin + n) * Cout + co] : 0.f;
  return ok;
}
__global__ void pack_bwd_kernel(const float* __restrict__ w, int taps, int Cin, int Cout,
                                float* __restrict__ dst, int Kpad, int Npad, int cout_total,
                                int co_off, int zero_first) {
  const size_t i = (size_t)blockIdx.x * blockDim.x + threadIdx.x;
  const size_t total = (size_t)Kpad * Npad;
  if (i >= total) return;
  float v;
  if (pack_bwd_value(i, w, taps, Cin, Cout, Npad, cout_total, co_off, &v) || zero_first) dst[i] = v;
}

__device__ __forceinline__ float pack_sub_value(size_t i, const float* __restrict__ w, int taps, int Cin_total, int Cout,
                                                int c_off, int Csub, int flip, int Npad) {
  const int tq = i & 3;
  const size_t rest = i >> 2;
  const int n = rest % Npad;
  const int k = (int)(rest / Npad) * 4 + tq;
  const int tp = k / Cout, co = k - tp * Cout;
  float v = 0.f;
  if (tp < taps && n < Csub) v = w[((size_t)(flip ? taps - 1 - tp : tp) * Cin_total + c_off + n) * Cout + co];
  return v;
}
__global__ void pack_sub_kernel(const float* __restrict__ w, int taps, int Cin_total, int Cout, int c_off,
                                int Csub, int flip, float* __restrict__ dst, int Kpad, int Npad) {
  const size_t i = (size_t)blockIdx.x * blockDim.x + threadIdx.x;
  const size_t total = (size_t)Kpad * Npad;
  if (i >= total) return;
  dst[i] = pack_sub_value(i, w, taps, Cin_total, Cout, c_off, Csub, flip, Npad);
}
int launch_pack_sub(hipStream_t st, const float* w, int taps, int Cin_total, int Cout, int c_off, int Csub,
                    int flip, float* dst, int Kpad, int Npad) {
  if (g_pack_rec) { g_pack_rec->push_back(PackJob{2, w, dst, {taps, Cin_total, Cout, c_off, Csub, flip, Npad, 0, 0}, (unsigned long long)Kpad * Npad, 0}); return 0; }
  const size_t total = (size_t)Kpad * Npad;
  ICS_LAUNCH(pack_sub_kernel, dim3((unsigned)((total + 255) / 256)), dim3(256), 0, st, w, taps, Cin_total,
                     Cout, c_off, Csub, flip, dst, Kpad, Npad);
  ICS_HIP(hipGetLastError());
  return 0;
}

int launch_pack_fwd(hipStream_t st, const float* w, int K, int N, float* dst, int Kpad, int Npad,
                    int k_off, int n_off, int zero_first, int cin_log, int cin_phys) {
  if (g_pack_rec) { g_pack_rec->push_back(PackJob{0, w, dst, {K, N, Npad, k_off, n_off, cin_log, cin_phys, 0, 0}, (unsigned long long)Kpad * Npad, 0}); return 0; }
  const size_t total = (size_t)Kpad * Npad;
  ICS_LAUNCH(pack_fwd_kernel, dim3((unsigned)((total + 255) / 256)), dim3(256), 0, st, w, K, N,
                     dst, Kpad, Npad, k_off, n_off, zero_first, cin_log, cin_phys);
  ICS_HIP(hipGetLastError());
  return 0;
}
int launch_pack_bwd(hipStream_t st, const float* w, int taps, int Cin, int Cout, float* dst,
                    int Kpad, int Npad, int cout_total, int co_off, int zero_first) {
  if (g_pack_rec) { g_pack_rec->push_back(PackJob{1, w, dst, {taps, Cin, Cout, Npad, cout_total, co_off, 0, 0, 0}, (unsigned long long)Kpad * Npad, 0}); return 0; }
  const size_t total = (size_t)Kpad * Npad;
  ICS_LAUNCH(pack_bwd_kernel, dim3((unsigned)((total + 255) / 256)), dim3(256), 0, st, w, taps,
                     Cin, Cout, dst, Kpad, Npad, cout_total, co_off, zero_first);
  ICS_HIP(hipGetLastError());
  return 0;
}

__device__ __forceinline__ void pack_wino_pair(size_t t, const float* __restrict__ w, int Cin_total, int Cout, int c_off,
                                               int Csub, int bwd, float* __restrict__ dst, int layout) {
  const int K = bwd ? Cout : Csub;
  if (layout == 2) {
    const int Nn = bwd ? Csub : Cout;
    const int k2 = (int)(t / ((size_t)4 * Nn)) * 4 + (int)(t & 3), n2 = (int)((t >> 2) % (size_t)Nn);
    float g2[27];
#pragma unroll
    for (int tap = 0; tap < 27; ++tap)
      g2[tap] = bwd ? w[((size_t)(26 - tap) * Cin_total + c_off + n2) * Cout + k2]
                    : w[((size_t)tap * Cin_total + c_off + k2) * Cout + n2];
    const size_t fs2 = (size_t)K * Nn;
    float* d2 = dst + t;
#pragma unroll
    for (int fz = 0; fz < 4; ++fz)
#pragma unroll
      for (int fy = 0; fy < 4; ++fy)
#pragma unroll
        for (int fx = 0; fx < 4; ++fx) {
          float acc = 0.f;
#pragma unroll
          for (int a = 0; a < 3; ++a) {
            const float ga = fz == 0 ? (a == 0 ? 1.f : 0.f) : fz == 3 ? (a == 2 ? 1.f : 0.f) : (fz == 2 && a == 1 ? -0.5f : 0.5f);
            if (ga == 0.f) continue;
#pragma unroll
            for (int b = 0; b < 3; ++b) {
              const float gb = fy == 0 ? (b == 0 ? 1.f : 0.f) : fy == 3 ? (b == 2 ? 1.f : 0.f) : (fy == 2 && b == 1 ? -0.5f : 0.5f);
              if (gb == 0.f) continue;
#pragma unroll
              for (int c = 0; c < 3; ++c) {
                const float gc = fx == 0 ? (c == 0 ? 1.f : 0.f) : fx == 3 ? (c == 2 ? 1.f : 0.f) : (fx == 2 && c == 1 ? -0.5f : 0.5f);
                if (gc == 0.f) continue;
                acc += (ga * gb * gc) * g2[(a * 3 + b) * 3 + c];
              }
            }
          }
// ... 223 lines not shown
```

icsg3d_amd/csrc/engine.hip:

```cpp
#include "common.h"
#include "elementwise.h"
#include "segment.h"
#include "scratch.h"
#include "voxelise.h"
#include "latent.h"
#include "tsne.h"
#include "render.h"
#include "monitor.h"
#include "feed.h"
#include "confusion.h"
#include "atomscore.h"
#include "../../include/icsg3d.h"

#include <rccl/rccl.h>
#include <roctracer/roctx.h>

#include <cmath>
#include <cstring>
#include <functional>
#include <map>
#include <memory>
#include <mutex>
#include <vector>

// ... 349 lines not shown
    Tensor t;
    t.name = name; t.dims = dims; t.trainable = trainable;
    t.count = 1;
    for (auto v : dims) t.count *= (size_t)v;
    if (trainable) { t.off = nparams; nparams += t.count; }
    tensors.push_back(t);
    tindex[name] = (int)tensors.size() - 1;
    return (int)tensors.size() - 1;
  }
  float* tp(int ti) const { return P + tensors[ti].off; }
  float* tg(int ti) const { return G + tensors[ti].off; }
  size_t rows(const ConvLayer& L, int B) const { return (size_t)B * L.S * L.S * L.S; }
};

static int padded_cin(int Cin) {
  if (Cin % 32 == 0 || Cin == 4 || Cin == 8 || Cin == 16) return Cin;
  return Cin < 4 ? 4 : (Cin < 8 ? 8 : (Cin < 16 ? 16 : round_up(Cin, 32)));
}

static ConvLayer* add_conv(Net& n, const std::string& name, int Cin, int Cout, int taps, int S, int pre_act,
                           int has_bn, int post_act, bool dense, bool register_params = true, bool pad_input = false) {
  auto L = std::make_unique<ConvLayer>();
  L->name = name; L->Cin = Cin; L->Cout = Cout; L->taps = taps; L->S = S;
  L->flags = n.flags;
  L->CinG = pad_input ? padded_cin(Cin) : Cin;
  L->pre_act = pre_act; L->has_bn = has_bn; L->post_act = post_act;
  L->Kpad = round_up(taps * L->CinG, 32); L->Npad = round_up(Cout, 32);
  L->Kpad_b = round_up(taps * Cout, 32); L->Npad_b = round_up(L->CinG, 32);
  if (register_params) {
    if (dense) L->t_w = n.add_tensor(name + "/kernel", {Cin, Cout}, true);
    else L->t_w = n.add_tensor(name + "/kernel", {taps == 27 ? 3 : 1, taps == 27 ? 3 : 1, taps == 27 ? 3 : 1, Cin, Cout}, true);
    L->t_b = n.add_tensor(name + "/bias", {Cout}, true);
    if (has_bn) {
      L->t_gamma = n.add_tensor(name + "/gamma", {Cout}, true);
      L->t_beta = n.add_tensor(name + "/beta", {Cout}, true);
    }
  }
  n.layers.push_back(std::move(L));
  return n.layers.back().get();
}

static int alloc_layer(Net& n, ConvLayer& L, bool need_bwd, bool pooled) {
  const size_t M = n.rows(L, n.maxB);
  ICS_TRY(n.alloc(&L.wp, (size_t)L.Kpad * L.Npad));
  ICS_TRY(n.alloc(&L.s, M * L.Cout));
  if (need_bwd) {
    ICS_TRY(n.alloc(&L.wf, (size_t)L.Kpad_b * L.Npad_b));
    ICS_TRY(n.alloc(&L.dy, M * L.Cout));
    ICS_TRY(n.alloc(&L.dA, M * L.CinG));
    ICS_TRY(n.alloc(&L.c1c2, (size_t)2 * L.Cout));
    if ((L.Cout & (L.Cout - 1)) == 0 || L.Cout % 4 == 0) {
      size_t rows = std::max((size_t)512, M / 128 + 1);
      for (int b = 1; b <= n.maxB; ++b) {
        LayerBwd lb{};
        lb.B = b; lb.S = L.S; lb.lgS = ilog2(L.S); lb.C = L.Cout;
        int rpb;
        rows = std::max(rows, (size_t)bn_bwd_num_blocks(lb, &rpb));
      }
      L.db_rows = rows;
      ICS_TRY(n.alloc(&L.db_partial, rows * L.Cout));
    }
    if (L.has_bn) { ICS_TRY(n.alloc(&L.xs, (size_t)2 * L.Cout)); ICS_TRY(n.alloc(&L.abc, (size_t)3 * L.Cout)); }
  }
  if (L.has_bn) {
    if (!n.bn_slab) {
      size_t tot = 0;
      for (auto& q : n.layers) if (q->has_bn) tot += 2 * (size_t)q->Cout;
      ICS_TRY(n.alloc(&n.bn_slab, tot));
      n.bn_slab_n = tot;
    }
    ICS_CHECK(n.bn_slab_used + 2 * (size_t)L.Cout <= n.bn_slab_n, "BN slab overflow");
    L.mm = n.bn_slab + n.bn_slab_used; L.mv = L.mm + L.Cout;
    n.bn_slab_used += 2 * (size_t)L.Cout;
    n.sync_cmax = std::max(n.sync_cmax, L.Cout);
    ICS_TRY(n.alloc(&L.mean, (size_t)L.Cout)); ICS_TRY(n.alloc(&L.rstd, (size_t)L.Cout));
    ICS_TRY(n.alloc(&L.scale, (size_t)L.Cout)); ICS_TRY(n.alloc(&L.shift, (size_t)L.Cout));
    int ti = n.add_tensor(L.name + "/moving_mean", {L.Cout}, false);
    n.tensors[ti].ptr = L.mm;
    ti = n.add_tensor(L.name + "/moving_var", {L.Cout}, false);
    n.tensors[ti].ptr = L.mv;
  }
  if (L.cond_fold) {
    ICS_TRY(n.alloc(&L.cond_T, (size_t)n.maxB * 27 * L.Cout));
  } else if (L.CinG != L.Cin) {
    ICS_TRY(n.alloc(&L.pad_in, M * L.CinG));
    if (need_bwd) ICS_TRY(n.alloc(&L.dw_phys, (size_t)L.taps * L.CinG * L.Cout));
  }
  if (pooled) {
    ICS_TRY(n.alloc(&L.pooled, M / 8 * L.Cout));
    ICS_TRY(n.alloc(&L.pool_idx, M / 8 * L.Cout));
    if (need_bwd && L.has_bn && L.Cout % 4 == 0) {
      ICS_TRY(n.alloc(&L.tie_mask, M / 8 * L.Cout));
      ICS_TRY(n.alloc(&L.tie_ssum, M / 8 * L.Cout));
      ICS_TRY(n.alloc(&L.bn_sums, (size_t)2 * L.Cout));
    }
  }
  return 0;
}

static ConvSrc src_plain(const float* p, int C) { return ConvSrc{p, nullptr, nullptr, C, 0, ACT_NONE, 0}; }
static ConvSrc src_layer(const ConvLayer& L, int up) {
  if (L.has_bn) return ConvSrc{L.s, L.scale, L.shift, L.Cout, up, L.post_act, 0};
  return ConvSrc{L.s, nullptr, nullptr, L.Cout, up, ACT_NONE, 0};
}

static ConvGeom geom_fwd(const ConvLayer& L, int B) {
  return ConvGeom{B, L.S, ilog2(L.S), L.CinG, L.Cout, L.taps, L.Kpad, L.Npad, L.flags};
}
static ConvGeom geom_bwd(const ConvLayer& L, int B) {
  return ConvGeom{B, L.S, ilog2(L.S), L.Cout, L.CinG, L.taps, L.Kpad_b, L.Npad_b, L.flags};
}

static ConvGeom geom_up_wgrad(const ConvLayer& L, int B) {
  return ConvGeom{B, L.S / 2, ilog2(L.S / 2), L.Cu, 27 * L.Cout, 1, round_up(L.Cu, 32), L.ldS, L.flags | (L.up8 ? CF_UP8 : 0)};
}
static ConvGeom geom_up_dgrad(const ConvLayer& L, int B) {
  return ConvGeom{B, L.S / 2, ilog2(L.S / 2), L.ldS, L.Cu, 1, L.ldS, round_up(L.Cu, 32), L.flags | (L.up8 ? CF_UP8 : 0)};
}
static ConvGeom geom_skip_wgrad(const ConvLayer& L, int B) {
  return ConvGeom{B, L.S, ilog2(L.S), L.Cs, L.Cout, L.taps, round_up(L.taps * L.Cs, 32), L.Npad, L.flags};
}
static ConvGeom geom_skip_dgrad(const ConvLayer& L, int B) {
  return ConvGeom{B, L.S, ilog2(L.S), L.Cout, L.Cs, L.taps, L.Kpad_b, round_up(L.Cs, 32), L.flags};
}
static ConvGeom geom_skip_fwd(const ConvLayer& L, int B) {
  return ConvGeom{B, L.S, ilog2(L.S), L.Cs, L.Cout, L.taps, round_up(L.taps * L.Cs, 32), L.Npad, L.flags};
}
static ConvGeom geom_par_fwd(const ConvLayer& L, int B) {
  return ConvGeom{B, L.S / 2, ilog2(L.S / 2), L.Cu, L.Cout, 8, 8 * L.Cu, L.Npad, L.flags};
}
static ConvSrc src_lowres(const ConvLayer& L) { ConvSrc u = L.src[L.nsrc - 1]; u.up = 0; return u; }

static bool up8_ok(const Net& n, const ConvLayer& L) {
  if (n.flags & CF_NO_UP8) return false;
  const size_t S3 = (size_t)(L.S / 2) * (L.S / 2) * (L.S / 2);
  if (L.Cout % 32 || L.Cu % 64 || !up8_shape_ok(L.S, L.Cout, (size_t)n.maxB * S3, n.maxB)) return false;
  for (int b = 1; b <= n.maxB; ++b)
    if (!conv_fwd_up8_tile_ok(geom_up_dgrad(L, b))) return false;
  return true;
}

constexpr size_t kUp125MinRows = 2048;
static bool up125_layer_ok(const Net& n, const ConvLayer& L) {
  if ((n.flags & CF_NO_UP125) || !L.up8 || n.side_on || n.sync() != nullptr) return false;
  if (!up125_shape_ok(L.S, L.Cout, L.Cu, n.maxB)) return false;
  if (n.flags & CF_FORCE_UP125) return true;
  return L.Cout % 128 == 0 && L.Cu % 128 == 0 && up125_geom(n.maxB, L.S, L.Cout, L.Cu).rows >= kUp125MinRows;
}
static bool up125_ok(const Net& n, const ConvLayer& L, int B) {
  if (!L.up125) return false;
  return (n.flags & CF_FORCE_UP125) || up125_geom(B, L.S, L.Cout, L.Cu).rows >= kUp125MinRows;
}
static size_t up125_splits(const ConvLayer& L, int B, Up125Splits* sp) {
  const int rows = (int)up125_geom(B, L.S, L.Cout, L.Cu).rows;
  size_t off = 0;
  for (int g = 0; g < 4; ++g) {
    const int nz = up125_group_classes(g), nb = 8 >> g;
    sp->off[g] = off;
    sp->ks[g] = wgrad_zbatch_splits(nz, rows, L.Cu, nb * L.Cout);
    off += (size_t)nz * sp->ks[g] * L.Cu * nb * L.Cout;
  }
  return off;
}

static int enable_split_up(Net& n, ConvLayer& L) {
  if (n.flags & CF_NO_UPSPLIT) return 0;
  const ConvSrc& up = L.src[L.nsrc - 1];
  const int Cs = L.nsrc == 2 ? L.src[0].C : 0;
  if (!up.up || (L.nsrc == 2 && L.src[0].up) || L.taps != 27 || L.S < 2 || L.CinG != L.Cin || Cs % 32 || up.C % 32 ||
      up.bcast || L.Cout % 4)
    return 0;
  L.split_up = true;
  L.Cs = Cs; L.Cu = up.C;
  L.ldS = round_up(27 * L.Cout, 32);
  const size_t M = n.rows(L, n.maxB);
  ICS_TRY(n.alloc(&L.w_up, (size_t)L.ldS * round_up(L.Cu, 32)));
  L.up8 = up8_ok(n, L);
  if (L.up8) {
    const size_t n8 = 8 * up8_volume_floats(n.maxB, L.S / 2, L.Cout);
    ICS_TRY(n.alloc(&L.dy8, n8));
    ICS_HIP(hipMemsetAsync(L.dy8, 0, n8 * sizeof(float), n.st));
  } else {
    ICS_TRY(n.alloc(&L.dyS, M / 8 * L.ldS));
    ICS_HIP(hipMemsetAsync(L.dyS, 0, M / 8 * L.ldS * sizeof(float), n.st));
  }
  L.up125 = up125_layer_ok(n, L);
  if (L.up125) {
    ICS_TRY(n.alloc(&L.w125, up125_weight_floats(L.Cout, L.Cu)));
    const size_t rows = up125_geom(n.maxB, L.S, L.Cout, L.Cu).rows;
    n.u125_P_n = std::max(n.u125_P_n, up125_pooled_floats(rows, L.Cout));
    n.u125_X_n = std::max(n.u125_X_n, up125_class_floats(rows, L.Cu));
    Up125Splits sp;
    for (int b = 1; b <= n.maxB; ++b)
      if (up125_ok(n, L, b)) n.u125_ws_n = std::max(n.u125_ws_n, up125_splits(L, b, &sp));
  }
  ICS_TRY(n.alloc(&L.dxl, M / 8 * L.Cu));
  ICS_TRY(n.alloc(&L.dw_up, (size_t)L.Cu * 27 * L.Cout));
  if (conv_up3_ok(geom_par_fwd(L, n.maxB), src_lowres(L)))
    ICS_TRY(n.alloc(&L.w_up3, conv_up3_weight_floats(L.Cu, L.Cout)));
  else if (L.Cs == 0 && conv_up3n_ok(geom_par_fwd(L, n.maxB), src_lowres(L)))
    ICS_TRY(n.alloc(&L.w_up3n, conv_up3n_weight_floats(L.Cu, L.Cout)));
  else
    ICS_TRY(n.alloc(&L.wp_par, (size_t)8 * 8 * L.Cu * L.Npad));
  if (L.Cs) {
    ICS_TRY(n.alloc(&L.wf_skip, (size_t)L.Kpad_b * round_up(L.Cs, 32)));
    ICS_TRY(n.alloc(&L.dA_skip, M * L.Cs));
    ICS_TRY(n.alloc(&L.wp_skip, (size_t)round_up(L.taps * L.Cs, 32) * L.Npad));
  }
  return 0;
}

static ConvGeom geom_wino_fwd(const ConvLayer& L, int B) { return L.split_up ? geom_skip_fwd(L, B) : geom_fwd(L, B); }
static ConvGeom geom_wino_bwd(const ConvLayer& L, int B) {
  if (L.split_up) return geom_skip_dgrad(L, B);
  ConvGeom g = geom_bwd(L, B);
  g.Cout = L.Cin;
  return g;
}
static int enable_wino(Net& n, ConvLayer& L, bool need_bwd) {
  if ((n.flags & CF_NO_WINO) || L.taps != 27 || L.pad_in || L.cond_fold || L.CinG != L.Cin) return 0;
  if (L.split_up ? L.Cs == 0 : L.nsrc != 1) return 0;
  const int K = L.split_up ? L.Cs : L.Cin;
  if (conv_wino_ok(geom_wino_fwd(L, n.maxB), L.src, 1)) {
    ICS_TRY(n.alloc(&L.ww, conv_wino_weight_floats(K, L.Cout)));
    L.ww_layout = conv_wino_layout(geom_wino_fwd(L, n.maxB));
  }
  const ConvSrc sdy = src_plain(nullptr, L.Cout);
  if (need_bwd && conv_wino_ok(geom_wino_bwd(L, n.maxB), &sdy, 1)) {
    ICS_TRY(n.alloc(&L.wwb, conv_wino_weight_floats(K, L.Cout)));
    L.wwb_layout = conv_wino_layout(geom_wino_bwd(L, n.maxB));
  }
  L.wino_w = need_bwd && conv_wino_wgrad_ok(L.split_up ? geom_skip_wgrad(L, n.maxB) : geom_fwd(L, n.maxB), L.src, 1);
  return 0;
}

static int enable_winog(Net& n, ConvLayer& L, bool need_bwd) {
  if (L.ww || L.taps != 27 || L.pad_in || L.cond_fold || L.CinG != L.Cin || L.split_up || L.nsrc != 1) return 0;
  const ConvGeom g = geom_fwd(L, n.maxB);
  if (!conv_winog_ok(g, L.src, 1)) return 0;
  size_t v, m, z;
  conv_winog_scratch_floats(g, &v, &m, &z);
  ICS_TRY(n.alloc(&L.wg, conv_winog_weight_floats(L.Cin, L.Cout)));
  ICS_TRY(n.alloc(&L.wg_v, v));
  ICS_TRY(n.alloc(&L.wg_m, m));
  if (need_bwd) {
    ConvGeom gb = geom_bwd(L, n.maxB);
    gb.Cout = L.Cin;
    const ConvSrc sdy = src_plain(nullptr, L.Cout);
    if (conv_winog_ok(gb, &sdy, 1)) ICS_TRY(n.alloc(&L.wgb, conv_winog_weight_floats(L.Cin, L.Cout)));
    L.wg_w = true;
    ICS_TRY(n.alloc(&L.wg_vt, (size_t)64 * n.maxB * 8 * L.Cin));
    ICS_TRY(n.alloc(&L.wg_z, z));
    ICS_TRY(n.alloc(&L.wg_du, (size_t)64 * L.Cin * L.Cout));
  }
  return 0;
}

static int alloc_workspaces(Net& n, bool need_bwd) {
  size_t stat = 0, bwd = 0, wg = 0, fw = 0;
  for (int b = 1; b <= n.maxB; ++b)
  for (auto& Lp : n.layers) {
    ConvLayer& L = *Lp;
    const size_t M = n.rows(L, b);
    const ConvGeom g = geom_fwd(L, b);
    const int rpb = std::min(conv_fwd_rows_per_block(g), 64);
    stat = std::max(stat, (M + rpb - 1) / rpb * 3 * (size_t)L.Npad);
    if (L.split_up) stat = std::max(stat, 8 * ((M / 8 + 63) / 64) * 3 * (size_t)L.Npad);
    fw = std::max(fw, conv_fwd_workspace_floats(g, L.src, L.nsrc));
    if (need_bwd) {
      const ConvSrc sdy = src_plain(L.dy, L.Cout);
      fw = std::max(fw, conv_fwd_workspace_floats(geom_bwd(L, b), &sdy, 1));
      if (L.split_up) {
        const ConvSrc sd = src_plain(L.up8 ? L.dy8 : L.dyS, L.ldS);
        fw = std::max(fw, conv_fwd_workspace_floats(geom_up_dgrad(L, b), &sd, 1));
        if (L.Cs) fw = std::max(fw, conv_fwd_workspace_floats(geom_skip_dgrad(L, b), &sdy, 1));
      }
      LayerBwd lb{};
      lb.B = b; lb.S = L.S; lb.lgS = ilog2(L.S); lb.C = L.Cout;
      if (&L != n.head) bwd = std::max(bwd, layer_bwd_workspace_floats(lb));
      wg = std::max(wg, conv_wgrad_workspace_floats(g, L.src, L.nsrc));
      if (L.wino_w)
        wg = std::max(wg, conv_wino_wgrad_workspace_floats(L.split_up ? geom_skip_wgrad(L, b) : g));
      if ((L.Cin == 1 || L.cond_fold) && (L.Cout == 16 || L.Cout == 32))
        wg = std::max(wg, conv_thin_c_wgrad_workspace_floats(g));
      if (L.split_up) {
        const ConvSrc lo = src_lowres(L);
        wg = std::max(wg, conv_wgrad_workspace_floats(geom_up_wgrad(L, b), &lo, 1));
        if (L.Cs) wg = std::max(wg, conv_wgrad_workspace_floats(geom_skip_wgrad(L, b), L.src, 1));
      }
    }
  }
  n.ws_stat_n = stat; n.ws_bwd_n = std::max(bwd, (size_t)4096 * 128); n.ws_wgrad_n = wg;
  ICS_TRY(n.alloc(&n.ws_stat, stat + 16));
  n.ws_fwd_n = std::max(fw, (size_t)768 * 64 * 64);
  ICS_TRY(n.alloc(&n.ws_fwd, n.ws_fwd_n + 16));
  if (need_bwd) {
    ICS_TRY(n.alloc(&n.ws_bwd, n.ws_bwd_n + 16));
    ICS_TRY(n.alloc(&n.ws_wgrad, wg + 16));
    if (n.u125_P_n && n.u125_P == nullptr) {
      ICS_TRY(n.alloc(&n.u125_P, n.u125_P_n));
      ICS_TRY(n.alloc(&n.u125_X, n.u125_X_n));
      ICS_TRY(n.alloc(&n.u125_O, n.u125_X_n));
      ICS_TRY(n.alloc(&n.u125_ws, n.u125_ws_n));
    }
    size_t b2 = 0;
    for (auto& Lp : n.layers)
      if (Lp->has_bn) b2 = std::max(b2, (size_t)2 * Lp->Npad * ((n.rows(*Lp, n.maxB) + 63) / 64));
    n.ws_bwd2_n = b2;
    ICS_TRY(n.alloc(&n.ws_bwd2, b2 + 16));
    size_t cls = 0; int cmax = 0;
    for (auto& Lp : n.layers)
      if (Lp->taps == 27 && Lp->S >= 3 && Lp->Cout % 4 == 0) {
        for (int b = 1; b <= n.maxB; ++b) cls = std::max(cls, conv_bnfuse_partial_floats(b, Lp->S, Lp->Cout));
        cmax = std::max(cmax, Lp->Cout);
      }
// ... 153 lines not shown
    }
  }
  if (L.pooled) {
    n.prof.begin(n.st, "pool_fwd", 0, 4.0 * M * L.Cout * 1.125);
    const bool ties = training && L.tie_mask != nullptr && (n.want_wgrad_inputs || n.want_tie_stats);
    L.tie_batch = ties ? B : 0;
    ICS_TRY(launch_pool_fwd(n.st, L.s, L.has_bn ? L.scale : nullptr, L.shift, L.has_bn ? L.post_act : ACT_NONE,
                            B, L.S, L.Cout, L.pooled, L.pool_idx, ties ? L.tie_mask : nullptr, ties ? L.tie_ssum : nullptr,
                            n.pool_ties_all));
    n.prof.end(n.st);
  }
  return 0;
}

__global__ void unpad_dw_kernel(const float* __restrict__ src, int Cin, int CinG, int N, size_t total,
                                float* __restrict__ dst) {
  const size_t i = (size_t)blockIdx.x * blockDim.x + threadIdx.x;
  if (i >= total) return;
  const size_t row = i / N, n = i - row * N;
  const size_t tap = row / Cin, ci = row - tap * Cin;
  dst[i] = src[(tap * CinG + ci) * N + n];
}
__global__ void axpy_strided_kernel(float* __restrict__ y, const float* __restrict__ x, size_t rows, int C, int ldx) {
  const size_t i = (size_t)blockIdx.x * blockDim.x + threadIdx.x;
  if (i >= rows * C) return;
  const size_t m = i / C, c = i - m * C;
  y[i] += x[m * ldx + c];
}
static void use_padded_input(ConvLayer& L) {
  if (L.CinG == L.Cin && !L.cond_fold) return;
  L.vsrc[0] = L.src[0]; L.vsrc[1] = L.src[1]; L.nvsrc = L.nsrc;
  L.src[0] = ConvSrc{L.pad_in, nullptr, nullptr, L.CinG, 0, ACT_NONE, 0};
  L.nsrc = 1;
}

static GradSrc gs_none() { return GradSrc{nullptr, 0, 0, GS_NONE, nullptr, nullptr}; }
static GradSrc gs_direct(const float* p, int ld, int off) { return GradSrc{p, ld, off, GS_DIRECT, nullptr, nullptr}; }
static GradSrc gs_up(const float* p, int ld, int off) { return GradSrc{p, ld, off, GS_UP, nullptr, nullptr}; }
static GradSrc gs_pool(const float* p, int ld, const ConvLayer& producer) {
  return GradSrc{p, ld, 0, GS_POOL, producer.pooled, producer.pool_idx};
}

static hipStream_t side_begin(Net& n) {
  if (!n.side_on || (n.prof.on && n.prof.filter.empty())) return n.st;
  (void)hipEventRecord(n.ev_fork, n.st);
  (void)hipStreamWaitEvent(n.st2, n.ev_fork, 0);
  n.side_dirty = true;
  return n.st2;
}
static int side_join(Net& n) {
  if (!n.side_dirty) return 0;
  ICS_HIP(hipEventRecord(n.ev_join, n.st2));
  ICS_HIP(hipStreamWaitEvent(n.st, n.ev_join, 0));
  n.side_dirty = false;
  return 0;
}

static BwdStat bwd_stat_for(Net& n, ConvLayer* next, int B) {
  BwdStat bs;
  if (next == nullptr || !next->has_bn || (n.flags & CF_NO_BWD_FOLD)) return bs;
  if ((size_t)2 * next->Npad * ((n.rows(*next, B) + 63) / 64) > n.ws_bwd2_n) return bs;
  bs.s = next->s; bs.mean = next->mean; bs.rstd = next->rstd; bs.scale = next->scale; bs.shift = next->shift;
  bs.partial = n.ws_bwd2; bs.post_act = next->post_act; bs.ld = next->Cout;
  return bs;
}
static void bwd_stat_done(ConvLayer* next, const BwdStat& bs, int blocks, int npad) {
  if (next == nullptr) return;
  next->bwd_pre_nblk = bs.partial ? blocks : 0;
  next->bwd_pre_ld = npad;
}

static bool skip_bnfuse_ok(const Net& n, const ConvLayer& L, int B) {
  const ConvLayer* P = L.skip_prod;
  if (P == nullptr || !L.split_up || L.Cs == 0 || (n.flags & CF_NO_DGRAD_BNFUSE) || n.sync() != nullptr || n.side_on) return false;
  if (!P->has_bn || P->pre_act != ACT_RELU || P->post_act != ACT_NONE || P->tie_mask == nullptr || P->xs == nullptr ||
      P->db_partial == nullptr || !P->pooled || P->Cout != L.Cs || L.src[0].p != P->s || L.src[0].scale == nullptr ||
      L.src[0].act != ACT_NONE || !n.want_wgrad_inputs || P->tie_batch != B)
    return false;
  if (!L.wino_w || !L.wwb || L.wwb_layout != 1) return false;
  if (n.rows(L, B) * (size_t)P->Cout * sizeof(float) < 2 * n.bnfuse_min_bytes) return false;
  const ConvGeom gw = geom_skip_wgrad(L, B), gd = geom_skip_dgrad(L, B);
  const ConvSrc sdy = src_plain(L.dy, L.Cout);
  return conv_bnfuse_ok(L.S, L.Cs, L.Cout) && conv_wino_wgrad_ok(gw, L.src, 1) && conv_wino_ok(gd, &sdy, 1) &&
         conv_bnfuse_partial_floats(B, L.S, L.Cout) <= n.ws_cls_n && L.Cs % 4 == 0 &&
         pool_bnfuse_partial_doubles(n.rows(L, B) / 8, P->Cout) <= n.ws_pool_n;
}
static int conv_grads_split_up(Net& n, ConvLayer& L, int B, ConvLayer* next) {
  const size_t M = n.rows(L, B);
  const double fl_skip = 2.0 * M * 27 * L.Cs * L.Cout, fl_up = 2.0 * (M / 8) * 27 * L.Cu * L.Cout;
  const bool skipfuse = skip_bnfuse_ok(n, L, B);
  ConvLayer* P = L.skip_prod;
  const float* dyp = L.up8 ? L.dy8 : L.dyS;
  const bool u125 = up125_ok(n, L, B);
  Up125Geom u5;
  Up125Splits sp5{};
  const double fl_up125 = 2.0 * (M / 64) * 125 * L.Cu * L.Cout;
  static thread_local std::string id125;
  auto mark125 = [&]() { id125 = std::string(conv_last_kernel_id()) + " UP125"; conv_set_last_kernel_id(id125.c_str()); };
  if (u125) {
    u5 = up125_geom(B, L.S, L.Cout, L.Cu);
    ICS_CHECK(up125_pooled_floats(u5.rows, L.Cout) <= n.u125_P_n && up125_class_floats(u5.rows, L.Cu) <= n.u125_X_n &&
                  up125_splits(L, B, &sp5) <= n.u125_ws_n, "up125 scratch smaller than the batch at hand");
    n.prof.begin(n.st, "pool125:" + L.name, 0, 4.0 * M * L.Cout * (1 + 125.0 / 64));
    ICS_TRY(launch_pool125(n.st, L.dy, B, L.S, L.Cout, n.u125_P, u5, (n.flags & CF_POOL125_V1) != 0));
  } else if (L.up8) {
    const double pr = (double)(L.S / 2 + 1) / (L.S / 2);
    n.prof.begin(n.st, "pool8:" + L.name, 0, 4.0 * M * L.Cout * (1 + pr * pr * pr));
    ICS_TRY(launch_pool8(n.st, L.dy, B, L.S, L.Cout, L.dy8, up8_geom(B, L.S / 2, ilog2(L.S / 2), L.Cout)));
  } else {
    n.prof.begin(n.st, "pool27:" + L.name, 0, 4.0 * M * L.Cout * (1 + 27.0 / 8));
    ICS_TRY(launch_pool27(n.st, L.dy, B, L.S, L.Cout, L.dyS, L.ldS));
  }
  n.prof.end(n.st);
  hipStream_t ws = side_begin(n);
  if (L.Cs) {
    const ConvGeom g = geom_skip_wgrad(L, B);
    n.prof.begin(ws, "conv_wgrad:" + L.name + ".skip|", fl_skip,
                 4.0 * (M * L.Cs + M * L.Cout + 27.0 * L.Cs * L.Cout));
    const bool wino = L.wino_w && conv_wino_wgrad_ok(g, L.src, 1);
    ConvSrc sx = L.src[0];
    if (skipfuse) { sx.scale = P->xs; sx.shift = P->xs + P->Cout; }
    if (wino)
      ICS_TRY(launch_conv_wgrad_wino(ws, g, sx, L.dy, L.Cout, n.tg(L.t_w), L.Cout, n.ws_wgrad, n.ws_wgrad_n,
                                     L.Cs, L.Cin, 0, 1));
    else
    ICS_TRY(launch_conv_wgrad(ws, g, L.src, 1, L.dy, L.Cout, n.tg(L.t_w), L.Cout, n.ws_wgrad, n.ws_wgrad_n, L.Cs,
                              L.Cin, 0, 1));
    n.prof.end(ws);
    n.prof.begin(ws, "wgrad_reduce_splits", 0, 0);
    if (wino)
      ICS_TRY(launch_conv_wgrad_wino(ws, g, sx, L.dy, L.Cout, n.tg(L.t_w), L.Cout, n.ws_wgrad, n.ws_wgrad_n,
                                     L.Cs, L.Cin, 0, 2));
    else
    ICS_TRY(launch_conv_wgrad(ws, g, L.src, 1, L.dy, L.Cout, n.tg(L.t_w), L.Cout, n.ws_wgrad, n.ws_wgrad_n, L.Cs,
                              L.Cin, 0, 2));
    n.prof.end(ws);
    if (skipfuse) {
      const bool pend = L.db_blocks > 0;
      n.prof.begin(ws, "bnfuse:" + L.name + ".skip", 0, 0);
      ICS_TRY(launch_conv_bnfuse(ws, L.dy, B, L.S, L.Cs, L.Cin, L.Cout, pend ? L.db_partial : n.tg(L.t_b), pend ? L.db_blocks : 1,
                                 n.tp(L.t_w), n.tg(L.t_w), n.tp(P->t_gamma), n.tp(P->t_beta), P->mean, P->rstd, P->scale,
                                 nullptr, nullptr, nullptr, nullptr, n.ws_cls, n.ws_cls_n, n.ws_R, P->bn_sums));
      n.prof.end(ws);
      P->deferred_skip = &L;
    }
  }
  if (u125) {
    const ConvSrc lo = src_lowres(L);
    const size_t rows = u5.rows;
    n.prof.begin(ws, "up125_xclass:" + L.name, 0, 4.0 * (M / 8 * L.Cu) * (1 + 27.0 / 8));
    ICS_TRY(launch_up125_xclass(ws, lo, n.u125_X, u5));
    n.prof.end(ws);
    n.prof.begin(ws, "conv_wgrad:" + L.name + ".up|", fl_up125, 4.0 * rows * (27.0 * L.Cu + 125.0 * L.Cout));
    for (int g = 0; g < 4; ++g)
      ICS_TRY(launch_wgrad_zbatch(ws, up125_group_classes(g), (int)rows, L.Cu, (8 >> g) * L.Cout,
                                  n.u125_X + (size_t)up125_group_slot0(g) * rows * L.Cu,
                                  n.u125_P + (size_t)up125_group_block0(g) * rows * L.Cout, n.u125_ws + sp5.off[g], sp5.ks[g]));
    mark125();
    n.prof.end(ws);
    n.prof.begin(ws, "wgrad_reduce_splits", 0, 0);
    ICS_TRY(launch_up125_contract(ws, n.u125_ws, sp5, L.dw_up, u5));
    ICS_TRY(launch_permute_up_dw(ws, L.dw_up, L.Cu, L.Cout, L.Cin, L.Cs, n.tg(L.t_w)));
    n.prof.end(ws);
  } else {
    const ConvGeom g = geom_up_wgrad(L, B);
    const ConvSrc lo = src_lowres(L);
    n.prof.begin(ws, "conv_wgrad:" + L.name + ".up|", fl_up,
                 4.0 * (M / 8 * L.Cu + M / 8 * 27.0 * L.Cout + 27.0 * L.Cu * L.Cout));
    ICS_TRY(launch_conv_wgrad(ws, g, &lo, 1, dyp, L.ldS, L.dw_up, 27 * L.Cout, n.ws_wgrad, n.ws_wgrad_n, 0, 0, 0, 1));
    n.prof.end(ws);
    n.prof.begin(ws, "wgrad_reduce_splits", 0, 0);
    ICS_TRY(launch_conv_wgrad(ws, g, &lo, 1, dyp, L.ldS, L.dw_up, 27 * L.Cout, n.ws_wgrad, n.ws_wgrad_n, 0, 0, 0, 2));
    ICS_TRY(launch_permute_up_dw(ws, L.dw_up, L.Cu, L.Cout, L.Cin, L.Cs, n.tg(L.t_w)));
    n.prof.end(ws);
  }
  if (L.Cs && !skipfuse) {
    const ConvGeom g = geom_skip_dgrad(L, B);
    ConvSrc sdy = src_plain(L.dy, L.Cout);
    n.prof.begin(n.st, "conv_dgrad:" + L.name + ".skip|", fl_skip,
                 4.0 * (M * L.Cs + M * L.Cout + 27.0 * L.Cs * L.Cout));
    if (L.wwb && conv_wino_ok(g, &sdy, 1))
      ICS_TRY(launch_conv_fwd_wino(n.st, g, sdy, L.wwb, nullptr, L.dA_skip, L.Cs, ACT_NONE, nullptr, nullptr, 0,
                                   L.wwb_layout));
    else
    ICS_TRY(launch_conv_fwd(n.st, g, &sdy, 1, L.wf_skip, nullptr, L.dA_skip, L.Cs, ACT_NONE, nullptr, nullptr, 0,
                            n.fws(), n.ws_fwd_n));
    n.prof.end(n.st);
  }
  if (u125) {
    const size_t rows = u5.rows;
    n.prof.begin(n.st, "conv_dgrad:" + L.name + ".up|", fl_up125, 4.0 * rows * (27.0 * L.Cu + 125.0 * L.Cout));
    for (int g = 0; g < 4; ++g)
      ICS_TRY(launch_gemm_zbatch(n.st, up125_group_classes(g), (int)rows, (8 >> g) * L.Cout, L.Cu,
                                 n.u125_P + (size_t)up125_group_block0(g) * rows * L.Cout,
                                 L.w125 + (size_t)up125_group_block0(g) * L.Cout * L.Cu,
                                 n.u125_O + (size_t)up125_group_slot0(g) * rows * L.Cu, L.flags));
    mark125();
    n.prof.end(n.st);
    n.prof.begin(n.st, "up125_combine:" + L.name, 0, 4.0 * (M / 8 * L.Cu) * (1 + 27.0 / 8));
    ICS_TRY(launch_up125_combine(n.st, n.u125_O, L.dxl, u5));
    n.prof.end(n.st);
    bwd_stat_done(next, BwdStat{}, 0, round_up(L.Cu, 32));
  } else {
    const ConvGeom g = geom_up_dgrad(L, B);
    ConvSrc sd = src_plain(dyp, L.ldS);
    n.prof.begin(n.st, "conv_dgrad:" + L.name + ".up|", fl_up,
                 4.0 * (M / 8 * L.Cu + M / 8 * 27.0 * L.Cout + 27.0 * L.Cu * L.Cout));
    const BwdStat bs = bwd_stat_for(n, next, B);
    int blocks = 0;
    ICS_TRY(launch_conv_fwd(n.st, g, &sd, 1, L.w_up, nullptr, L.dxl, L.Cu, ACT_NONE, nullptr, nullptr, 0, n.fws(),
                            n.ws_fwd_n, &bs, &blocks));
    bwd_stat_done(next, bs, blocks, g.Npad);
    n.prof.end(n.st);
  }
  return 0;
}

static int colsum_push(Net& n, const float* partial, int nblk, int C, float* out);
static bool dgrad_bnfuse_ok(const Net& n, const ConvLayer& L, const ConvLayer* next, int B, bool need_dA, bool param_grads) {
  if (next == nullptr || !need_dA || !param_grads || (n.flags & CF_NO_DGRAD_BNFUSE) || n.sync() != nullptr || n.side_on)
    return false;
  if (!next->has_bn || next->pre_act != ACT_RELU || next->post_act != ACT_NONE || next->xs == nullptr ||
      next->db_partial == nullptr || next->dy == nullptr)
    return false;
  if (L.split_up || L.nsrc != 1 || L.taps != 27 || !L.wino_w || !L.wwb || L.CinG != L.Cin ||
      L.Cin != next->Cout || L.src[0].p != next->s || L.src[0].scale == nullptr || L.src[0].act != ACT_NONE || L.dw_phys)
    return false;
  if (n.rows(L, B) * (size_t)next->Cout * sizeof(float) < n.bnfuse_min_bytes) return false;
  const ConvGeom g = geom_fwd(L, B);
  ConvGeom gb = geom_bwd(L, B);
  gb.Cout = L.Cin;
  const ConvSrc sdy = src_plain(L.dy, L.Cout);
  return conv_bnfuse_ok(L.S, L.Cin, L.Cout) && conv_wino_wgrad_ok(g, L.src, 1) && conv_wino_ok(gb, &sdy, 1) &&
         conv_bnfuse_partial_floats(B, L.S, L.Cout) <= n.ws_cls_n && L.Cin % 4 == 0;
}
static int conv_grads_from_dy(Net& n, ConvLayer& L, int B, bool need_dA, bool param_grads, ConvLayer* next) {
  if (L.split_up && need_dA && param_grads) return conv_grads_split_up(n, L, B, next);
  if (L.split_up) next = nullptr;
  const ConvGeom g = geom_fwd(L, B);
  const size_t M = n.rows(L, B);
  const bool bnfuse = dgrad_bnfuse_ok(n, L, next, B, need_dA, param_grads);
  if (param_grads) {
    hipStream_t ws = side_begin(n);
    n.prof.begin(ws, "conv_wgrad:" + L.name + "|", 2.0 * M * L.taps * L.Cin * L.Cout,
                 4.0 * (M * L.Cin + M * L.Cout + (double)L.taps * L.Cin * L.Cout));
    float* dw = L.dw_phys ? L.dw_phys : n.tg(L.t_w);
    const bool thin1 = L.pad_in && L.nvsrc == 1 && L.Cin == 1 && conv_thin_c_ok(g, L.vsrc[0], 1, 1) && L.Cout % 4 == 0;
    if (L.cond_fold) {
      const ConvSrc& cs = L.vsrc[1];
      const int C0 = L.vsrc[0].C;
      ICS_TRY(launch_conv_wgrad_thin_c(ws, g, L.vsrc[0], L.dy, L.Cout, n.tg(L.t_w), L.Cout, L.Cin, n.ws_wgrad,
                                       n.ws_wgrad_n, 0));
      ICS_TRY(launch_cond_wgrad(ws, L.dy, B, L.S, L.Cout, cs.p, C0, cs.C, cs.bcast, L.Cin, n.tg(L.t_w), n.ws_dbl,
                                n.ws_dbl_n));
      conv_set_last_kernel_id(L.Cout == 32 ? "conv_thin_c_wgrad_kernel<32> + cond_wgrad_kernel"
                                           : "conv_thin_c_wgrad_kernel<16> + cond_wgrad_kernel");
      n.prof.end(ws);
    } else if (thin1) {
      ICS_TRY(launch_conv_wgrad_thin_c(ws, g, L.vsrc[0], L.dy, L.Cout, n.tg(L.t_w), L.Cout, L.Cin, n.ws_wgrad,
                                       n.ws_wgrad_n, 1));
      n.prof.end(ws);
      n.prof.begin(ws, "wgrad_reduce_splits", 0, 0);
      ICS_TRY(launch_conv_wgrad_thin_c(ws, g, L.vsrc[0], L.dy, L.Cout, n.tg(L.t_w), L.Cout, L.Cin, n.ws_wgrad,
                                       n.ws_wgrad_n, 2));
      n.prof.end(ws);
    } else if (L.wg_w && L.wg_vt_batch == B && conv_winog_wgrad_ok(g, L.src, L.nsrc)) {
      ICS_TRY(launch_conv_wgrad_winog(ws, g, L.wg_vt, L.dy, L.Cout, dw, L.Cout, 0, 0, L.wg_z, L.wg_du));
      n.prof.end(ws);
    } else if (L.wino_w && !L.split_up && conv_wino_wgrad_ok(g, L.src, L.nsrc)) {
      ConvSrc sx = L.src[0];
      if (bnfuse) {
        sx.scale = next->xs; sx.shift = next->xs + next->Cout;
      }
      ICS_TRY(launch_conv_wgrad_wino(ws, g, sx, L.dy, L.Cout, dw, L.Cout, n.ws_wgrad, n.ws_wgrad_n, 0, 0, 0, 1));
      n.prof.end(ws);
      n.prof.begin(ws, "wgrad_reduce_splits", 0, 0);
      ICS_TRY(launch_conv_wgrad_wino(ws, g, sx, L.dy, L.Cout, dw, L.Cout, n.ws_wgrad, n.ws_wgrad_n, 0, 0, 0, 2));
      n.prof.end(ws);
      if (bnfuse) {
        const bool pend = L.db_blocks > 0;
        n.prof.begin(ws, "bnfuse:" + L.name, 0, 0);
        ICS_TRY(launch_conv_bnfuse(ws, L.dy, B, L.S, L.Cin, L.Cin, L.Cout, pend ? L.db_partial : n.tg(L.t_b), pend ? L.db_blocks : 1,
                                   n.tp(L.t_w), dw, n.tp(next->t_gamma), n.tp(next->t_beta), next->mean, next->rstd,
                                   next->scale, next->abc, next->c1c2, n.tg(next->t_gamma), n.tg(next->t_beta), n.ws_cls,
                                   n.ws_cls_n, n.ws_R));
        n.prof.end(ws);
      }
    } else {
    ICS_TRY(launch_conv_wgrad(ws, g, L.src, L.nsrc, L.dy, L.Cout, dw, L.Cout, n.ws_wgrad, n.ws_wgrad_n, 0, 0, 0, 1));
    n.prof.end(ws);
    n.prof.begin(ws, "wgrad_reduce_splits", 0, 0);
    ICS_TRY(launch_conv_wgrad(ws, g, L.src, L.nsrc, L.dy, L.Cout, dw, L.Cout, n.ws_wgrad, n.ws_wgrad_n, 0, 0, 0, 2));
    if (L.dw_phys) {
      const size_t cnt = (size_t)L.taps * L.Cin * L.Cout;
      ICS_LAUNCH(unpad_dw_kernel, dim3((unsigned)((cnt + 255) / 256)), dim3(256), 0, ws, L.dw_phys, L.Cin,
                         L.CinG, L.Cout, cnt, n.tg(L.t_w));
      ICS_HIP(hipGetLastError());
    }
    n.prof.end(ws);
    }
  }
  if (need_dA) {
    ConvGeom gb = geom_bwd(L, B);
    gb.Cout = L.Cin;
    ConvSrc sdy = src_plain(L.dy, L.Cout);
    n.prof.begin(n.st, "conv_dgrad:" + L.name + "|", 2.0 * M * L.taps * L.Cin * L.Cout,
                 4.0 * (M * L.Cin + M * L.Cout + (double)L.taps * L.Cin * L.Cout));
    int blocks = 0;
    if (bnfuse) {
      BwdStat ba{};
      ba.s = next->s; ba.ld = next->Cout; ba.abc = next->abc; ba.db_partial = next->db_partial;
      ICS_TRY(launch_conv_fwd_wino(n.st, gb, sdy, L.wwb, nullptr, next->dy, next->Cout, ACT_NONE, nullptr, nullptr, 0,
                                   L.wwb_layout, &ba, &blocks));
      n.prof.end(n.st);
      ICS_CHECK(blocks > 0, "fused BatchNorm-backward apply: the backward-data launch did not take it");
      ICS_CHECK((size_t)blocks <= next->db_rows, "bias-gradient partial buffer too small for this batch");
      next->dy_ready = true;
      next->db_blocks = 0;
      ICS_TRY(colsum_push(n, next->db_partial, blocks, next->Cout, n.tg(next->t_b)));
      next->db_blocks = blocks;
      return 0;
    }
    const BwdStat bs = bwd_stat_for(n, next, B);
    if (L.wwb && !L.split_up && conv_wino_ok(gb, &sdy, 1))
      ICS_TRY(launch_conv_fwd_wino(n.st, gb, sdy, L.wwb, nullptr, L.dA, L.CinG, ACT_NONE, nullptr, nullptr, 0,
                                   L.wwb_layout, &bs, &blocks));
    else if (L.wgb && conv_winog_ok(gb, &sdy, 1))
      ICS_TRY(launch_conv_fwd_winog(n.st, gb, sdy, L.wgb, nullptr, L.dA, L.CinG, ACT_NONE, nullptr, nullptr, L.wg_v, L.wg_m,
                                    nullptr));
    else {
      if (L.split_up && L.wf_stale) {
        ICS_TRY(launch_pack_bwd(n.st, n.tp(L.t_w), L.taps, L.Cin, L.Cout, L.wf, L.Kpad_b, L.Npad_b, L.Cout, 0, 1));
        L.wf_stale = false;
      }
      ICS_TRY(launch_conv_fwd(n.st, gb, &sdy, 1, L.wf, nullptr, L.dA, L.CinG, ACT_NONE, nullptr, nullptr, 0, n.fws(),
                              n.ws_fwd_n, &bs, &blocks));
    }
    bwd_stat_done(next, bs, blocks, gb.Npad);
    n.prof.end(n.st);
  }
  return 0;
}

static int colsum_push(Net& n, const float* partial, int nblk, int C, float* out) {
  ColsumJobs& J = n.colsum;
  if (J.n == 24) { ICS_TRY(launch_colsum_batch(n.st, J)); J.n = 0; }
  if (J.n == 0) J.blk0[0] = 0;
  J.partial[J.n] = partial; J.out[J.n] = out; J.nblk[J.n] = nblk; J.C[J.n] = C;
  J.blk0[J.n + 1] = J.blk0[J.n] + colsum_blocks(C);
// ... 2953 lines not shown
```

Measured before the change: 1185.

## Merge four up125 class-group GEMM launches into one ragged grouped launch

```diff
diff --git a/icsg3d_amd/csrc/common.h b/icsg3d_amd/csrc/common.h
--- a/icsg3d_amd/csrc/common.h
+++ b/icsg3d_amd/csrc/common.h
@@ -9,6 +9,7 @@
 
 #include "up8.h"
 #include "up125.h"
+#include "up125_ragged.h"
 
 namespace ics {
 
@@ -115,6 +116,7 @@
   CF_FORCE_UP125 = 1 << 28,
   CF_POOL125_V1 = 1 << 29,
   CF_ZBATCH = 1 << 20,
+  CF_UP125_SPLIT_LAUNCH = 1 << 30,
 };
 int conv_flags_from_env();
 
@@ -220,6 +222,9 @@
 int launch_gemm_zbatch(hipStream_t st, int nz, int M, int K, int N, const float* A, const float* Wp, float* out, int flags);
 int wgrad_zbatch_splits(int nz, int M, int K, int N);
 int launch_wgrad_zbatch(hipStream_t st, int nz, int M, int K, int N, const float* x, const float* dy, float* ws, int ksplit);
+int launch_gemm_ragged(hipStream_t st, const RaggedGroupDesc* d, int n, int M, int N, const float* A, const float* Wp, float* out,
+                       int flags);
+int launch_wgrad_ragged(hipStream_t st, const RaggedGroupDesc* d, int n, int M, int K, const float* x, const float* dy, float* ws);
 int launch_pack_up125(hipStream_t st, const float* w, int Cin_total, int N, int c_off, int Cu, float* dst);
 int launch_pack_up125_pieces(hipStream_t st, const float* w, int Cin_total, int N, int c_off, int Cu, float* dst);
 bool conv_up3n_ok(const ConvGeom& g, const ConvSrc& s0);
diff --git a/icsg3d_amd/csrc/conv_igemm.hip b/icsg3d_amd/csrc/conv_igemm.hip
--- a/icsg3d_amd/csrc/conv_igemm.hip
+++ b/icsg3d_amd/csrc/conv_igemm.hip
@@ -64,6 +64,7 @@
   if (getenv("ICSG3D_NO_UP125")) f |= CF_NO_UP125;
   if (getenv("ICSG3D_FORCE_UP125")) f |= CF_FORCE_UP125;
   if (getenv("ICSG3D_POOL125_V1")) f |= CF_POOL125_V1;
+  if (getenv("ICSG3D_UP125_SPLIT_LAUNCH")) f |= CF_UP125_SPLIT_LAUNCH;
   { const char* e = getenv("ICSG3D_UP3_BIG_MIN_WG"); if (e && *e && strtoul(e, nullptr, 10) <= 1) f |= CF_UP3_BIG_ALWAYS; }
   return f;
 }
@@ -186,7 +187,8 @@
                                                         const float* __restrict__ bias,
                                                         float* __restrict__ out, int ldo, int pre_act,
                                                         float* __restrict__ stat_partial, int gridM,
-                                                        int gridN, int accumulate, BwdStat bs, Up8Geom u8) {
+                                                        int gridN, int accumulate, BwdStat bs, Up8Geom u8,
+                                                        RaggedGroups rg) {
   constexpr int BM = WM * TM * 32, BN = WN * TN * 32;
   constexpr int B_FLOATS = 32 * BN;
   constexpr int RA = BM / 32;
@@ -201,21 +203,32 @@
   const int t = threadIdx.x, lane = t & 63, wave = t >> 6;
   const int wm = wave / WN, wn = wave % WN;
   const int li = lane & 31, lh = lane >> 5;
-  const int sw = xcd_swizzle(blockIdx.x, gridM * gridN);
-  const int mb = sw / gridN, nb = sw % gridN;
+  int sw = xcd_swizzle(blockIdx.x, gridM * gridN);
+  int mb = sw / gridN, nb = sw % gridN;
   const int S = g.S, lg = g.lgS;
   const int M = g.B << (3 * lg);
-  const int n0 = nb * BN;
-  const int nchunks = g.Kpad >> 5;
-  const int cpt = (VEC && !THIN) ? (g.Cin >> 5) : 1;
+  int n0 = nb * BN;
+  int nchunks = g.Kpad >> 5;
+  int cpt = (VEC && !THIN) ? (g.Cin >> 5) : 1;
   const int cls = PAR ? (int)blockIdx.y : 0;
   const int pz = cls >> 2, py = (cls >> 1) & 1, px = cls & 1;
   if (PAR) wp += (size_t)cls * g.Kpad * g.Npad;
   const bool zbatch = (g.flags & CF_ZBATCH) != 0;
   if (zbatch) {
-    s0.p += (size_t)blockIdx.z * (size_t)M * (size_t)s0.C;
-    wp += (size_t)blockIdx.z * (size_t)g.Kpad * (size_t)g.Npad;
-    out += (size_t)blockIdx.z * (size_t)M * (size_t)ldo;
+    if (rg.n != 0) {
+      const RaggedGemmWg w = ragged_gemm_wg(rg, blockIdx.x, M, g.Npad);
+      g.Cin = w.K; g.Kpad = w.K; s0.C = w.K;
+      s0.p += w.a_off; wp += w.w_off; out += w.o_off;
+      sw = xcd_swizzle(w.local, gridM * gridN);
+      mb = sw / gridN; nb = sw % gridN;
+      n0 = nb * BN;
+      nchunks = w.K >> 5;
+      cpt = (VEC && !THIN) ? (w.K >> 5) : 1;
+    } else {
+      s0.p += (size_t)blockIdx.z * (size_t)M * (size_t)s0.C;
+      wp += (size_t)blockIdx.z * (size_t)g.Kpad * (size_t)g.Npad;
+      out += (size_t)blockIdx.z * (size_t)M * (size_t)ldo;
+    }
   }
   const int zsplit = zbatch ? 1 : (int)gridDim.z, zidx = zbatch ? 0 : (int)blockIdx.z;
 
@@ -826,7 +839,7 @@
 static int launch_fwd_cfg(hipStream_t st, const ConvGeom& g, const ConvSrc& s0, const ConvSrc& s1,
                           const float* wp, const float* bias, float* out, int ldo, int pre_act,
                           float* stat_partial, int* rows_per_block, int accumulate = 0, int ksplit = 1,
-                          const BwdStat* bwd = nullptr) {
+                          const BwdStat* bwd = nullptr, const RaggedGroups* ragged = nullptr) {
   constexpr int BM = WM * TM * 32, BN = WN * TN * 32;
   const int M = g.B << (3 * g.lgS);
   const int gridM = (M + BM - 1) / BM, gridN = g.Npad / BN;
@@ -851,8 +864,10 @@
   if (FOLD) bs_arg = *bwd;
   Up8Geom u8;
   if (UP8) u8 = up8_geom(g.B, g.S, g.lgS, g.Cin / 27);
-  ICS_LAUNCH(kern, dim3(gridM * gridN, PAR ? 8 : 1, ksplit), dim3(256), lds, st, g, s0, s1, wp, bias, out, ldo,
-                     pre_act, stat_partial, gridM, gridN, accumulate, bs_arg, u8);
+  RaggedGroups rg;
+  if (ragged) rg = *ragged;
+  ICS_LAUNCH(kern, ragged ? dim3(rg.end[rg.n - 1]) : dim3(gridM * gridN, PAR ? 8 : 1, ksplit), dim3(256), lds, st, g, s0, s1,
+                     wp, bias, out, ldo, pre_act, stat_partial, gridM, gridN, accumulate, bs_arg, u8, rg);
   ICS_HIP(hipGetLastError());
   return 0;
 }
@@ -892,11 +907,32 @@
 #ifndef ICS_ZB_BIG
 #define ICS_ZB_BIG 1
 #endif
-  if (ICS_ZB_BIG && M % 128 == 0 && N % 128 == 0 && (long)(M / 128) * (N / 128) * nz >= 512)
+  if (ICS_ZB_BIG && zbatch_gemm_big_tile(nz, M, N))
     return launch_fwd_cfg<2, 2, 2, 2, true, 0, false, false, false, false, false, true, false>(
         st, g, s0, s1, Wp, nullptr, out, N, ACT_NONE, nullptr, nullptr, 0, nz);
   return launch_fwd_cfg<2, 2, 1, 1, true, 0, false, false, false, false, false, true, false>(
       st, g, s0, s1, Wp, nullptr, out, N, ACT_NONE, nullptr, nullptr, 0, nz);
+}
+int launch_gemm_ragged(hipStream_t st, const RaggedGroupDesc* d, int n, int M, int N, const float* A, const float* Wp, float* out,
+                       int flags) {
+  ICS_CHECK(n >= 1 && n <= RAGGED_MAX_GROUPS && M >= 1 && N % 64 == 0, "ragged GEMM: 1..4 groups, N % 64 required");
+  int kmax = 0;
+  for (int g = 0; g < n; ++g) {
+    ICS_CHECK(d[g].classes >= 1 && d[g].dim >= 32 && d[g].dim % 32 == 0, "ragged GEMM: K % 32 required");
+    kmax = std::max(kmax, d[g].dim);
+  }
+  ICS_CHECK((size_t)M * (size_t)std::max(kmax, N) < ((size_t)1 << 30), "ragged GEMM: matrix too large for 32-bit offsets");
+  const bool big = ICS_ZB_BIG && ragged_gemm_big_tile(d, M, N);
+  const int bt = big ? 128 : 64;
+  const RaggedGroups rg = ragged_gemm_table(d, n, M, N, bt, bt);
+  ICS_CHECK((size_t)rg.end[n - 1] < ((size_t)1 << 31), "ragged GEMM: grid too large");
+  const ConvGeom g{M, 1, 0, d[0].dim, N, 1, d[0].dim, N, flags | CF_ZBATCH};
+  const ConvSrc s0{A, nullptr, nullptr, d[0].dim, 0, ACT_NONE, 0}, s1{};
+  if (big)
+    return launch_fwd_cfg<2, 2, 2, 2, true, 0, false, false, false, false, false, true, false>(
+        st, g, s0, s1, Wp, nullptr, out, N, ACT_NONE, nullptr, nullptr, 0, 1, nullptr, &rg);
+  return launch_fwd_cfg<2, 2, 1, 1, true, 0, false, false, false, false, false, true, false>(
+      st, g, s0, s1, Wp, nullptr, out, N, ACT_NONE, nullptr, nullptr, 0, 1, nullptr, &rg);
 }
 
 int conv_fwd_rows_per_block(const ConvGeom& g) {
@@ -1899,7 +1935,7 @@
                                                           const float* __restrict__ dy, int ldy,
                                                           int n_load,
                                                           float* __restrict__ ws, int ktiles,
-                                                          int ntiles, int rows_per_split, Up8Geom u8) {
+                                                          int ntiles, int rows_per_split, Up8Geom u8, RaggedGroups rg) {
   constexpr int KT = WM * TM * 32, NT = WN * TN * 32;
   constexpr int A_FLOATS = 32 * KT, D_FLOATS = 32 * NT;
   constexpr int AF4 = KT / 4, ATOT = 32 * AF4, APASS = ATOT / 256;
@@ -1915,13 +1951,21 @@
   const int S = g.S, lg = g.lgS;
   const int M = g.B << (3 * lg);
   const int K = g.taps * g.Cin;
+  int bid = blockIdx.x;
   if (ZB) {
-    s0.p += (size_t)blockIdx.y * (size_t)M * (size_t)s0.C;
-    dy += (size_t)blockIdx.y * (size_t)M * (size_t)ldy;
-    ws += (size_t)blockIdx.y * (size_t)(gridDim.x / (unsigned)(ktiles * ntiles)) * (size_t)K * (size_t)g.Cout;
-  }
-
-  int bid = blockIdx.x;
+    if (rg.n != 0) {
+      const RaggedWgradWg w = ragged_wgrad_wg(rg, blockIdx.x, M, K, ktiles);
+      g.Cout = w.N; ldy = w.N; n_load = w.N;
+      ntiles = w.ntiles; rows_per_split = w.rows_per_split;
+      s0.p += w.x_off; dy += w.dy_off; ws += w.ws_off;
+      bid = w.local;
+    } else {
+      s0.p += (size_t)blockIdx.y * (size_t)M * (size_t)s0.C;
+      dy += (size_t)blockIdx.y * (size_t)M * (size_t)ldy;
+      ws += (size_t)blockIdx.y * (size_t)(gridDim.x / (unsigned)(ktiles * ntiles)) * (size_t)K * (size_t)g.Cout;
+    }
+  }
+
   const int nt_i = bid % ntiles; bid /= ntiles;
   const int kt_i = bid % ktiles; bid /= ktiles;
   const int split = bid;
@@ -2691,7 +2735,8 @@
 template <int WM, int WN, int TM, int TN, bool VEC, bool DYVEC, bool AFF = true, bool UP = true, bool THIN = false,
           int ABL = 0, bool UP8 = false, bool ZB = false>
 static int launch_wgrad_cfg(hipStream_t st, const ConvGeom& g, const ConvSrc& s0, const ConvSrc& s1,
-                            const float* dy, int ldy, int n_load, float* ws, const WgradPlan& p, int nz = 1) {
+                            const float* dy, int ldy, int n_load, float* ws, const WgradPlan& p, int nz = 1,
+                            const RaggedGroups* ragged = nullptr) {
   constexpr int KT = WM * TM * 32, NT = WN * TN * 32;
   const size_t lds = (size_t)2 * 32 * (KT + NT) * sizeof(float);
   auto kern = conv_wgrad_kernel<WM, WN, TM, TN, VEC, DYVEC, AFF, UP, THIN, ABL, UP8, ZB>;
@@ -2709,8 +2754,10 @@
   g_last_kernel_id = id.c_str();
   Up8Geom u8;
   if (UP8) u8 = up8_geom(g.B, g.S, g.lgS, g.Cout / 27);
-  ICS_LAUNCH(kern, dim3(p.ktiles * p.ntiles * p.ksplit, ZB ? nz : 1), dim3(256), lds, st, g, s0, s1, dy,
-                     ldy, n_load, ws, p.ktiles, p.ntiles, p.rows_per_split, u8);
+  RaggedGroups rg;
+  if (ZB && ragged) rg = *ragged;
+  ICS_LAUNCH(kern, rg.n ? dim3(rg.end[rg.n - 1]) : dim3(p.ktiles * p.ntiles * p.ksplit, ZB ? nz : 1), dim3(256), lds, st, g, s0,
+                     s1, dy, ldy, n_load, ws, p.ktiles, p.ntiles, p.rows_per_split, u8, rg);
   ICS_HIP(hipGetLastError());
   return 0;
 }
@@ -2894,11 +2941,7 @@
   return 0;
 }
 
-int wgrad_zbatch_splits(int nz, int M, int K, int N) {
-  const long base = (long)((K + 127) / 128) * ((N + 127) / 128) * nz;
-  const long ks_max = std::max<long>(1, M / 256);
-  return (int)std::max<long>(1, std::min<long>(std::min<long>(512 / base, ks_max), 512));
-}
+int wgrad_zbatch_splits(int nz, int M, int K, int N) { return zbatch_wgrad_splits(nz, M, K, N); }
 int launch_wgrad_zbatch(hipStream_t st, int nz, int M, int K, int N, const float* x, const float* dy, float* ws, int ksplit) {
   ICS_CHECK(nz >= 1 && nz <= 65535 && M >= 1 && K % 32 == 0 && N % 4 == 0 && ksplit >= 1, "z-batched wgrad: K % 32, N % 4 required");
   ICS_CHECK((size_t)M * (size_t)std::max(K, N) < ((size_t)1 << 30), "z-batched wgrad: matrix too large for 32-bit offsets");
@@ -2916,6 +2959,31 @@
   p.ksplit = ksplit;
   return launch_wgrad_cfg<2, 2, 2, 2, true, true, false, false, false, 0, false, true>(st, g, s0, s1, dy, N, N, ws, p, nz);
 }
+int launch_wgrad_ragged(hipStream_t st, const RaggedGroupDesc* d, int n, int M, int K, const float* x, const float* dy, float* ws) {
+  ICS_CHECK(n >= 1 && n <= RAGGED_MAX_GROUPS && M >= 1 && K % 32 == 0, "ragged wgrad: 1..4 groups, K % 32 required");
+  int nmax = 0;
+  for (int g = 0; g < n; ++g) {
+    ICS_CHECK(d[g].classes >= 1 && d[g].dim >= 4 && d[g].dim % 4 == 0 && d[g].ksplit >= 1, "ragged wgrad: N % 4 required");
+    const int rps = ragged_rows_per_split(M, d[g].ksplit);
+    ICS_CHECK((M + rps - 1) / rps <= d[g].ksplit, "ragged wgrad: split plan");
+    nmax = std::max(nmax, d[g].dim);
+  }
+  ICS_CHECK((size_t)M * (size_t)std::max(K, nmax) < ((size_t)1 << 30), "ragged wgrad: matrix too large for 32-bit offsets");
+  const RaggedGroups rg = ragged_wgrad_table(d, n, M, K);
+  ICS_CHECK((size_t)rg.end[n - 1] < ((size_t)1 << 31), "ragged wgrad: grid too large");
+  const int N0 = d[0].dim;
+  const ConvGeom g{M, 1, 0, K, N0, 1, K, (N0 + 31) / 32 * 32, 0};
+  const ConvSrc s0{x, nullptr, nullptr, K, 0, ACT_NONE, 0};
+  ConvSrc s1 = s0;
+  s1.C = 0;
+  WgradPlan p;
+  p.vec = true; p.thin = false;
+  p.kt = 128; p.nt = 128;
+  p.ktiles = (K + 127) / 128; p.ntiles = rg.ntiles[0];
+  p.rows_per_split = rg.rows_per_split[0];
+  p.ksplit = d[0].ksplit;
+  return launch_wgrad_cfg<2, 2, 2, 2, true, true, false, false, false, 0, false, true>(st, g, s0, s1, dy, N0, N0, ws, p, 1, &rg);
+}
 
 __device__ __forceinline__ bool pack_fwd_value(size_t i, const float* __restrict__ w, int K, int N, int Npad, int k_off,
                                                int n_off, int cin_log, int cin_phys, float* v) {
diff --git a/icsg3d_amd/csrc/engine.hip b/icsg3d_amd/csrc/engine.hip
--- a/icsg3d_amd/csrc/engine.hip
+++ b/icsg3d_amd/csrc/engine.hip
@@ -525,15 +525,7 @@
   return (n.flags & CF_FORCE_UP125) || up125_geom(B, L.S, L.Cout, L.Cu).rows >= kUp125MinRows;
 }
 static size_t up125_splits(const ConvLayer& L, int B, Up125Splits* sp) {
-  const int rows = (int)up125_geom(B, L.S, L.Cout, L.Cu).rows;
-  size_t off = 0;
-  for (int g = 0; g < 4; ++g) {
-    const int nz = up125_group_classes(g), nb = 8 >> g;
-    sp->off[g] = off;
-    sp->ks[g] = wgrad_zbatch_splits(nz, rows, L.Cu, nb * L.Cout);
-    off += (size_t)nz * sp->ks[g] * L.Cu * nb * L.Cout;
-  }
-  return off;
+  return up125_split_plan((int)up125_geom(B, L.S, L.Cout, L.Cu).rows, L.Cu, L.Cout, sp->off, sp->ks);
 }
 
 static int enable_split_up(Net& n, ConvLayer& L) {
@@ -993,10 +985,15 @@
     ICS_TRY(launch_up125_xclass(ws, lo, n.u125_X, u5));
     n.prof.end(ws);
     n.prof.begin(ws, "conv_wgrad:" + L.name + ".up|", fl_up125, 4.0 * rows * (27.0 * L.Cu + 125.0 * L.Cout));
-    for (int g = 0; g < 4; ++g)
-      ICS_TRY(launch_wgrad_zbatch(ws, up125_group_classes(g), (int)rows, L.Cu, (8 >> g) * L.Cout,
-                                  n.u125_X + (size_t)up125_group_slot0(g) * rows * L.Cu,
-                                  n.u125_P + (size_t)up125_group_block0(g) * rows * L.Cout, n.u125_ws + sp5.off[g], sp5.ks[g]));
+    RaggedGroupDesc gd[4];
+    up125_wgrad_groups((int)rows, L.Cu, L.Cout, sp5.off, sp5.ks, gd);
+    if (n.flags & CF_UP125_SPLIT_LAUNCH) {
+      for (int g = 0; g < 4; ++g)
+        ICS_TRY(launch_wgrad_zbatch(ws, gd[g].classes, (int)rows, L.Cu, gd[g].dim, n.u125_X + gd[g].a_off, n.u125_P + gd[g].b_off,
+                                    n.u125_ws + gd[g].o_off, gd[g].ksplit));
+    } else {
+      ICS_TRY(launch_wgrad_ragged(ws, gd, 4, (int)rows, L.Cu, n.u125_X, n.u125_P, n.u125_ws));
+    }
     mark125();
     n.prof.end(ws);
     n.prof.begin(ws, "wgrad_reduce_splits", 0, 0);
@@ -1031,11 +1028,15 @@
   if (u125) {
     const size_t rows = u5.rows;
     n.prof.begin(n.st, "conv_dgrad:" + L.name + ".up|", fl_up125, 4.0 * rows * (27.0 * L.Cu + 125.0 * L.Cout));
-    for (int g = 0; g < 4; ++g)
-      ICS_TRY(launch_gemm_zbatch(n.st, up125_group_classes(g), (int)rows, (8 >> g) * L.Cout, L.Cu,
-                                 n.u125_P + (size_t)up125_group_block0(g) * rows * L.Cout,
-                                 L.w125 + (size_t)up125_group_block0(g) * L.Cout * L.Cu,
-                                 n.u125_O + (size_t)up125_group_slot0(g) * rows * L.Cu, L.flags));
+    RaggedGroupDesc gd[4];
+    up125_gemm_groups((int)rows, L.Cu, L.Cout, gd);
+    if (n.flags & CF_UP125_SPLIT_LAUNCH) {
+      for (int g = 0; g < 4; ++g)
+        ICS_TRY(launch_gemm_zbatch(n.st, gd[g].classes, (int)rows, gd[g].dim, L.Cu, n.u125_P + gd[g].a_off, L.w125 + gd[g].b_off,
+                                   n.u125_O + gd[g].o_off, L.flags));
+    } else {
+      ICS_TRY(launch_gemm_ragged(n.st, gd, 4, (int)rows, L.Cu, n.u125_P, L.w125, n.u125_O, L.flags));
+    }
     mark125();
     n.prof.end(n.st);
     n.prof.begin(n.st, "up125_combine:" + L.name, 0, 4.0 * (M / 8 * L.Cu) * (1 + 27.0 / 8));
diff --git a/icsg3d_amd/csrc/hoststub/up125_ragged_check.cpp b/icsg3d_amd/csrc/hoststub/up125_ragged_check.cpp
--- /dev/null
+++ b/icsg3d_amd/csrc/hoststub/up125_ragged_check.cpp
@@ -0,0 +1,128 @@
+#include "../up125_ragged.h"
+
+#include <cstdio>
+#include <map>
+#include <tuple>
+#include <vector>
+
+static int g_fail = 0;
+#define CHECK(cond, ...)                                 \
+  do {                                                   \
+    if (!(cond)) {                                       \
+      if (g_fail < 20) {                                 \
+        fprintf(stderr, "up125_ragged_check FAILED: ");  \
+        fprintf(stderr, __VA_ARGS__);                    \
+        fprintf(stderr, "\n");                           \
+      }                                                  \
+      ++g_fail;                                          \
+    }                                                    \
+  } while (0)
+
+static unsigned check_wgrad(int B, int S, int N, int Cu) {
+  const Up125Geom u = up125_geom(B, S, N, Cu);
+  const int rows = (int)u.rows, M = rows, K = Cu, ktiles = (K + 127) / 128;
+  unsigned long long off[4];
+  int ks[4];
+  const size_t ws_floats = up125_split_plan(rows, Cu, N, off, ks);
+  RaggedGroupDesc d[4];
+  up125_wgrad_groups(rows, Cu, N, off, ks, d);
+  const RaggedGroups t = ragged_wgrad_table(d, 4, M, K);
+  const size_t x_floats = up125_class_floats(u.rows, Cu), p_floats = up125_pooled_floats(u.rows, N);
+  std::map<std::tuple<int, int, int, int, int>, int> hit;
+  unsigned bid = 0;
+  for (int g = 0; g < 4; ++g) {
+    const int nz = up125_group_classes(g), Ng = (8 >> g) * N, ntiles = (Ng + 127) / 128;
+    const int rps = ((M + ks[g] - 1) / ks[g] + 31) / 32 * 32;
+    CHECK((M + rps - 1) / rps <= ks[g], "wgrad group %d: %d splits of %d rows do not cover %d rows", g, ks[g], rps, M);
+    const unsigned gx = (unsigned)(ktiles * ntiles * ks[g]);
+    for (int y = 0; y < nz; ++y)
+      for (unsigned x = 0; x < gx; ++x, ++bid) {
+        int b = (int)x;
+        const int nt = b % ntiles; b /= ntiles;
+        const int kt = b % ktiles; b /= ktiles;
+        const int split = b;
+        const unsigned long long xo = (unsigned long long)up125_group_slot0(g) * rows * Cu + (unsigned long long)y * M * K;
+        const unsigned long long dyo = (unsigned long long)up125_group_block0(g) * rows * N + (unsigned long long)y * M * Ng;
+        const unsigned long long wso = off[g] + (unsigned long long)y * (gx / (unsigned)(ktiles * ntiles)) * K * Ng;
+        CHECK(bid < t.end[t.n - 1], "wgrad: workgroup %u past the ragged grid of %u", bid, t.end[t.n - 1]);
+        const RaggedWgradWg w = ragged_wgrad_wg(t, bid, M, K, ktiles);
+        CHECK(w.g == g && w.cls == y && w.local == (int)x, "wgrad %u: (group %d, class %d, local %d), four launches (%d, %d, %u)",
+              bid, w.g, w.cls, w.local, g, y, x);
+        CHECK(w.nt == nt && w.kt == kt && w.split == split, "wgrad %u: tile (%d, %d) split %d, four launches (%d, %d) %d", bid,
+              w.nt, w.kt, w.split, nt, kt, split);
+        CHECK(w.N == Ng && w.ntiles == ntiles && w.ksplit == ks[g] && w.rows_per_split == rps,
+              "wgrad %u: N %d tiles %d splits %d rows %d, four launches %d %d %d %d", bid, w.N, w.ntiles, w.ksplit,
+              w.rows_per_split, Ng, ntiles, ks[g], rps);
+        CHECK(w.x_off == xo && w.dy_off == dyo && w.ws_off == wso, "wgrad %u: offsets %llu %llu %llu, four launches %llu %llu %llu",
+              bid, w.x_off, w.dy_off, w.ws_off, xo, dyo, wso);
+        CHECK(w.x_off + (size_t)M * K <= x_floats && w.dy_off + (size_t)M * w.N <= p_floats &&
+                  w.ws_off + (size_t)w.ksplit * K * w.N <= ws_floats && w.split < w.ksplit && w.kt < ktiles && w.nt < w.ntiles,
+              "wgrad %u: a matrix outside its buffer", bid);
+        ++hit[std::make_tuple(w.g, w.cls, w.kt, w.nt, w.split)];
+      }
+  }
+  CHECK(bid == t.end[t.n - 1], "wgrad: %u workgroups in four launches, %u in the ragged grid", bid, t.end[t.n - 1]);
+  CHECK(hit.size() == bid, "wgrad: %zu distinct (class, tile, split) for %u workgroups", hit.size(), bid);
+  for (const auto& h : hit) CHECK(h.second == 1, "wgrad: a (class, tile, split) hit %d times", h.second);
+  return bid;
+}
+
+static unsigned check_gemm(int B, int S, int N, int Cu, int bt) {
+  const Up125Geom u = up125_geom(B, S, N, Cu);
+  const int rows = (int)u.rows, M = rows;
+  RaggedGroupDesc d[4];
+  up125_gemm_groups(rows, Cu, N, d);
+  const RaggedGroups t = ragged_gemm_table(d, 4, M, Cu, bt, bt);
+  const size_t o_floats = up125_class_floats(u.rows, Cu), p_floats = up125_pooled_floats(u.rows, N);
+  const size_t w_floats = up125_weight_floats(N, Cu);
+  const unsigned tiles = (unsigned)(((M + bt - 1) / bt) * (Cu / bt));
+  std::map<std::tuple<int, int, int>, int> hit;
+  unsigned bid = 0;
+  for (int g = 0; g < 4; ++g) {
+    const int nz = up125_group_classes(g), Kg = (8 >> g) * N;
+    for (int z = 0; z < nz; ++z)
+      for (unsigned x = 0; x < tiles; ++x, ++bid) {
+        const unsigned long long ao = (unsigned long long)up125_group_block0(g) * rows * N + (unsigned long long)z * M * Kg;
+        const unsigned long long wo = (unsigned long long)up125_group_block0(g) * N * Cu + (unsigned long long)z * Kg * Cu;
+        const unsigned long long oo = (unsigned long long)up125_group_slot0(g) * rows * Cu + (unsigned long long)z * M * Cu;
+        CHECK(bid < t.end[t.n - 1], "gemm: workgroup %u past the ragged grid of %u", bid, t.end[t.n - 1]);
+        const RaggedGemmWg w = ragged_gemm_wg(t, bid, M, Cu);
+        CHECK(w.g == g && w.cls == z && w.local == (int)x && w.K == Kg, "gemm %u: (group %d, class %d, tile %d, K %d), four launches (%d, %d, %u, %d)",
+              bid, w.g, w.cls, w.local, w.K, g, z, x, Kg);
+        CHECK(w.a_off == ao && w.w_off == wo && w.o_off == oo, "gemm %u: offsets %llu %llu %llu, four launches %llu %llu %llu", bid,
+              w.a_off, w.w_off, w.o_off, ao, wo, oo);
+        CHECK(w.a_off + (size_t)M * w.K <= p_floats && w.w_off + (size_t)w.K * Cu <= w_floats && w.o_off + (size_t)M * Cu <= o_floats,
+              "gemm %u: a matrix outside its buffer", bid);
+        ++hit[std::make_tuple(w.g, w.cls, w.local)];
+      }
+  }
+  CHECK(bid == t.end[t.n - 1], "gemm: %u workgroups in four launches, %u in the ragged grid", bid, t.end[t.n - 1]);
+  CHECK(hit.size() == bid, "gemm: %zu distinct (class, tile) for %u workgroups", hit.size(), bid);
+  for (const auto& h : hit) CHECK(h.second == 1, "gemm: a (class, tile) hit %d times", h.second);
+  return bid;
+}
+
+int main() {
+  const int shapes[6][4] = {{2, 8, 128, 128}, {3, 16, 32, 64}, {3, 16, 64, 64}, {4, 32, 128, 128}, {32, 32, 128, 128}, {32, 16, 256, 256}};
+  for (const auto& s : shapes) {
+    const int B = s[0], S = s[1], N = s[2], Cu = s[3];
+    CHECK(up125_shape_ok(S, N, Cu, B), "shape (B %d, S %d, N %d, Cu %d) refused", B, S, N, Cu);
+    const int rows = (int)up125_geom(B, S, N, Cu).rows;
+    const unsigned wg = check_wgrad(B, S, N, Cu);
+    RaggedGroupDesc d[4];
+    up125_gemm_groups(rows, Cu, N, d);
+    const bool big = ragged_gemm_big_tile(d, rows, Cu);
+    const unsigned gm = check_gemm(B, S, N, Cu, big ? 128 : 64);
+    if (rows % 128 == 0 && Cu % 128 == 0) check_gemm(B, S, N, Cu, big ? 64 : 128);
+    printf("up125_ragged_check: B %d S %d Cout %d Cu %d: %d tile rows, backward-weight %u workgroups, backward-data %u on %s tiles\n", B, S, N,
+           Cu, rows, wg, gm, big ? "128 x 128" : "64 x 64");
+    if (B == 32 && S == 32) CHECK(wg == 1560, "c17: %u backward-weight workgroups, 1560 expected", wg);
+    if (B == 32 && S == 16) CHECK(wg == 1312, "c15: %u backward-weight workgroups, 1312 expected", wg);
+  }
+  if (g_fail) {
+    fprintf(stderr, "up125_ragged_check: %d checks failed\n", g_fail);
+    return 1;
+  }
+  printf("up125_ragged_check: ok\n");
+  return 0;
+}
diff --git a/icsg3d_amd/csrc/up125_ragged.h b/icsg3d_amd/csrc/up125_ragged.h
--- /dev/null
+++ b/icsg3d_amd/csrc/up125_ragged.h
@@ -0,0 +1,147 @@
+#pragma once
+#include "up125.h"
+
+enum { RAGGED_MAX_GROUPS = 4 };
+
+struct RaggedGroupDesc {
+  int classes = 0, dim = 0, ksplit = 1;
+  unsigned long long a_off = 0, b_off = 0, o_off = 0;
+};
+
+struct RaggedGroups {
+  int n = 0;
+  unsigned end[RAGGED_MAX_GROUPS] = {};
+  unsigned per_class[RAGGED_MAX_GROUPS] = {};
+  int dim[RAGGED_MAX_GROUPS] = {};
+  int ntiles[RAGGED_MAX_GROUPS] = {};
+  int ksplit[RAGGED_MAX_GROUPS] = {};
+  int rows_per_split[RAGGED_MAX_GROUPS] = {};
+  unsigned long long a_off[RAGGED_MAX_GROUPS] = {}, b_off[RAGGED_MAX_GROUPS] = {}, o_off[RAGGED_MAX_GROUPS] = {};
+};
+
+template <class T>
+ICS_UP125_F T ragged_sel(const T (&a)[RAGGED_MAX_GROUPS], int g) {
+  return g == 0 ? a[0] : (g == 1 ? a[1] : (g == 2 ? a[2] : a[3]));
+}
+ICS_UP125_F int ragged_group(const RaggedGroups& t, unsigned bid) {
+  return (int)(bid >= t.end[0]) + (int)(bid >= t.end[1]) + (int)(bid >= t.end[2]);
+}
+
+struct RaggedWgradWg {
+  int g, cls, local;
+  int nt, kt, split;
+  int N, ntiles, ksplit, rows_per_split;
+  unsigned long long x_off, dy_off, ws_off;
+};
+ICS_UP125_F RaggedWgradWg ragged_wgrad_wg(const RaggedGroups& t, unsigned bid, int M, int K, int ktiles) {
+  RaggedWgradWg w;
+  w.g = ragged_group(t, bid);
+  const unsigned first = w.g == 0 ? 0u : (w.g == 1 ? t.end[0] : (w.g == 2 ? t.end[1] : t.end[2]));
+  const unsigned per = ragged_sel(t.per_class, w.g), r = bid - first;
+  w.cls = (int)(r / per);
+  w.local = (int)(r - (unsigned)w.cls * per);
+  w.N = ragged_sel(t.dim, w.g);
+  w.ntiles = ragged_sel(t.ntiles, w.g);
+  w.ksplit = ragged_sel(t.ksplit, w.g);
+  w.rows_per_split = ragged_sel(t.rows_per_split, w.g);
+  int b = w.local;
+  w.nt = b % w.ntiles; b /= w.ntiles;
+  w.kt = b % ktiles; b /= ktiles;
+  w.split = b;
+  w.x_off = ragged_sel(t.a_off, w.g) + (unsigned long long)w.cls * (unsigned long long)M * (unsigned long long)K;
+  w.dy_off = ragged_sel(t.b_off, w.g) + (unsigned long long)w.cls * (unsigned long long)M * (unsigned long long)w.N;
+  w.ws_off = ragged_sel(t.o_off, w.g) +
+             (unsigned long long)w.cls * (unsigned long long)w.ksplit * (unsigned long long)K * (unsigned long long)w.N;
+  return w;
+}
+
+struct RaggedGemmWg {
+  int g, cls, local, K;
+  unsigned long long a_off, w_off, o_off;
+};
+ICS_UP125_F RaggedGemmWg ragged_gemm_wg(const RaggedGroups& t, unsigned bid, int M, int N) {
+  RaggedGemmWg w;
+  w.g = ragged_group(t, bid);
+  const unsigned first = w.g == 0 ? 0u : (w.g == 1 ? t.end[0] : (w.g == 2 ? t.end[1] : t.end[2]));
+  const unsigned per = ragged_sel(t.per_class, w.g), r = bid - first;
+  w.cls = (int)(r / per);
+  w.local = (int)(r - (unsigned)w.cls * per);
+  w.K = ragged_sel(t.dim, w.g);
+  w.a_off = ragged_sel(t.a_off, w.g) + (unsigned long long)w.cls * (unsigned long long)M * (unsigned long long)w.K;
+  w.w_off = ragged_sel(t.b_off, w.g) + (unsigned long long)w.cls * (unsigned long long)w.K * (unsigned long long)N;
+  w.o_off = ragged_sel(t.o_off, w.g) + (unsigned long long)w.cls * (unsigned long long)M * (unsigned long long)N;
+  return w;
+}
+
+ICS_UP125_HD int ragged_rows_per_split(int M, int ksplit) { return ((M + ksplit - 1) / ksplit + 31) / 32 * 32; }
+inline RaggedGroups ragged_finish(RaggedGroups t, int n) {
+  t.n = n;
+  for (int g = 1; g < n; ++g) t.end[g] += t.end[g - 1];
+  for (int g = n; g < RAGGED_MAX_GROUPS; ++g) {
+    t.end[g] = t.end[n - 1]; t.per_class[g] = 1; t.ntiles[g] = 1; t.ksplit[g] = 1; t.rows_per_split[g] = 32;
+  }
+  return t;
+}
+inline RaggedGroups ragged_wgrad_table(const RaggedGroupDesc* d, int n, int M, int K) {
+  RaggedGroups t;
+  const int ktiles = (K + 127) / 128;
+  for (int g = 0; g < n; ++g) {
+    t.dim[g] = d[g].dim;
+    t.ntiles[g] = (d[g].dim + 127) / 128;
+    t.ksplit[g] = d[g].ksplit;
+    t.rows_per_split[g] = ragged_rows_per_split(M, d[g].ksplit);
+    t.per_class[g] = (unsigned)(ktiles * t.ntiles[g] * d[g].ksplit);
+    t.end[g] = (unsigned)d[g].classes * t.per_class[g];
+    t.a_off[g] = d[g].a_off; t.b_off[g] = d[g].b_off; t.o_off[g] = d[g].o_off;
+  }
+  return ragged_finish(t, n);
+}
+inline RaggedGroups ragged_gemm_table(const RaggedGroupDesc* d, int n, int M, int N, int bm, int bn) {
+  RaggedGroups t;
+  for (int g = 0; g < n; ++g) {
+    t.dim[g] = d[g].dim;
+    t.ntiles[g] = 1; t.ksplit[g] = 1; t.rows_per_split[g] = 32;
+    t.per_class[g] = (unsigned)(((M + bm - 1) / bm) * (N / bn));
+    t.end[g] = (unsigned)d[g].classes * t.per_class[g];
+    t.a_off[g] = d[g].a_off; t.b_off[g] = d[g].b_off; t.o_off[g] = d[g].o_off;
+  }
+  return ragged_finish(t, n);
+}
+ICS_UP125_HD bool zbatch_gemm_big_tile(int nz, int M, int N) {
+  return M % 128 == 0 && N % 128 == 0 && (long)(M / 128) * (N / 128) * nz >= 512;
+}
+inline bool ragged_gemm_big_tile(const RaggedGroupDesc* d, int M, int N) { return zbatch_gemm_big_tile(d[0].classes, M, N); }
+
+ICS_UP125_HD int zbatch_wgrad_splits(int nz, int M, int K, int N) {
+  const long base = (long)((K + 127) / 128) * ((N + 127) / 128) * nz;
+  const long ks_max = M / 256 > 1 ? M / 256 : 1;
+  long ks = 512 / base < ks_max ? 512 / base : ks_max;
+  ks = ks < 512 ? ks : 512;
+  return (int)(ks > 1 ? ks : 1);
+}
+inline size_t up125_split_plan(int rows, int Cu, int N, unsigned long long off[4], int ks[4]) {
+  size_t o = 0;
+  for (int g = 0; g < 4; ++g) {
+    const int nz = up125_group_classes(g), nb = 8 >> g;
+    off[g] = o;
+    ks[g] = zbatch_wgrad_splits(nz, rows, Cu, nb * N);
+    o += (size_t)nz * ks[g] * Cu * nb * N;
+  }
+  return o;
+}
+inline void up125_wgrad_groups(int rows, int Cu, int N, const unsigned long long off[4], const int ks[4], RaggedGroupDesc d[4]) {
+  for (int g = 0; g < 4; ++g) {
+    d[g].classes = up125_group_classes(g); d[g].dim = (8 >> g) * N; d[g].ksplit = ks[g];
+    d[g].a_off = (unsigned long long)up125_group_slot0(g) * rows * Cu;
+    d[g].b_off = (unsigned long long)up125_group_block0(g) * rows * N;
+    d[g].o_off = off[g];
+  }
+}
+inline void up125_gemm_groups(int rows, int Cu, int N, RaggedGroupDesc d[4]) {
+  for (int g = 0; g < 4; ++g) {
+    d[g].classes = up125_group_classes(g); d[g].dim = (8 >> g) * N; d[g].ksplit = 1;
+    d[g].a_off = (unsigned long long)up125_group_block0(g) * rows * N;
+    d[g].b_off = (unsigned long long)up125_group_block0(g) * N * Cu;
+    d[g].o_off = (unsigned long long)up125_group_slot0(g) * rows * Cu;
+  }
+}
```

New measurement: 1190, median of 6. No clear change (+0.4%).
